# eric-downes/tianshou_marl

Measured on AMD Instinct MI355X. Metric: env-steps/sec (n_env x n_agent) incl. PPO update, simple_spread N=3, higher is better.
Workload: dtype f32; 1 GPU; simple_spread_v3 N=3 shared PPO, num_envs=1024 per GPU, obs 18, A=5, T=25, MLP 64-64; minibatch=4096, repeat=1, dispatch=per_agent, parallelism=env-shard x1

## Files before the change

tianshou_marl_amd/csrc/mlp_fused.hip:

```cpp
#include "common.h"
#include "mlp_tile.h"
#include "philox.h"

extern long long *g_tsm_stamps;

namespace {

template <int H, int DS = 0>
__global__ __launch_bounds__(NT) void policy_forward_kernel(
    const float *__restrict__ P, const float *__restrict__ img, Dims d_arg, const float *__restrict__ obs, int64_t B,
    uint64_t seed,
    uint64_t offset, const uint64_t *__restrict__ offset_dev, int mode ,
    float *__restrict__ logits_out,
    float *__restrict__ value_out, int32_t *__restrict__ act_io, float *__restrict__ logp_out) {
    extern __shared__ float lds[];
    const Dims d = DS ? dims_const(DS, 5) : d_arg;
    const Lay<H> ly(d, false);
    if (img) stage_image<H>(lds, ly, img);
    else stage_weights<H>(lds, ly, d, P);
    if (offset_dev) offset += *offset_dev;
    const int64_t n_tiles = (B + R - 1) / R;
    float xr[kXRegs];
    if ((int64_t)blockIdx.x < n_tiles) prefetch_tile_x(xr, d, obs, nullptr, 0, (int64_t)blockIdx.x * R, B);
    for (int64_t t = blockIdx.x; t < n_tiles; t += gridDim.x) {
        const int64_t row0 = t * R;
        __syncthreads();
        commit_tile_x(lds, ly.X, d, xr);
        if (t + gridDim.x < n_tiles) prefetch_tile_x(xr, d, obs, nullptr, 0, (t + gridDim.x) * R, B);
        __syncthreads();
        tile_forward<H>(lds, ly, d);
        if (logits_out) {
            for (int e = threadIdx.x; e < R * d.A; e += NT) {
                const int r = e / d.A, c = e - r * d.A;
                if (row0 + r < B) logits_out[(row0 + r) * d.A + c] = lds[ly.OUT + r * ly.ldo + c];
            }
        }
        if (threadIdx.x < R && row0 + threadIdx.x < B) {
            const int r = threadIdx.x;
            const int64_t i = row0 + r;
            const float *lg = lds + ly.OUT + r * ly.ldo;
            if (value_out) value_out[i] = lg[16];
            if (mode != 0) {
                float m = -INFINITY;
                int arg = 0;
                for (int j = 0; j < d.A; ++j) if (lg[j] > m) { m = lg[j]; arg = j; }
                float s = 0.f;
                for (int j = 0; j < d.A; ++j) s += expf(lg[j] - m);
                int a = arg;
                if (mode == 1) {
                    const float u = tsm_philox_uniform(seed, offset + (uint64_t)i) * s;
                    float c = 0.f;
                    a = d.A - 1;
                    for (int j = 0; j < d.A; ++j) { c += expf(lg[j] - m); if (u < c) { a = j; break; } }
                } else if (mode == 3) {
                    a = act_io[i];
                }
                if (mode != 3) act_io[i] = a;
                if (logp_out) logp_out[i] = lg[a] - (m + logf(s));
            }
        }
    }
}

struct LossCfg {
    float eps_clip, dual_clip, vf_coef, ent_coef;
    int value_clip, adv_norm, kind;
};

template <int H>
__global__ __launch_bounds__(NT) void ppo_update_kernel(
    const float *__restrict__ P, const float *__restrict__ img, Dims d, const float *__restrict__ obs,
    const int32_t *__restrict__ act,
    const float *__restrict__ logp_old, const float *__restrict__ adv, const float *__restrict__ returns,
    const float *__restrict__ v_s_old, const int64_t *__restrict__ perm, int64_t first, int64_t M,
    const float *__restrict__ adv_stats, LossCfg cfg, float *__restrict__ slabs,
    double *__restrict__ loss_partial, int64_t *__restrict__ opt_step_dev, long long *stamps) {
#define USTAMP(k) do { if (stamps && blockIdx.x == 0 && threadIdx.x == 0) stamps[k] = (long long)wall_clock64(); } while (0)
    extern __shared__ float lds[];
    USTAMP(0);
    if (stamps && threadIdx.x == 0 && blockIdx.x < 256) stamps[64 + 2 * blockIdx.x] = (long long)wall_clock64();
    if (opt_step_dev && blockIdx.x == 0 && threadIdx.x == 0) *opt_step_dev += 1;
    const Lay<H> ly(d, true);
    const POff<H> po(d.D, d.A);
    const int64_t n_tiles = (M + R - 1) / R;
    float xr[kXRegs];
    struct RowIn { int a_idx; float adv, logp_old, ret, v_old; } rin;
    auto row_id = [&](int64_t row0) -> int64_t {
        const int64_t i = row0 + (threadIdx.x >> 4);
        return i < M ? (perm ? perm[i] : first + i) : -1;
    };
    auto prefetch_row = [&](int64_t src) {
        rin.a_idx = 0; rin.adv = 0.f; rin.logp_old = 0.f; rin.ret = 0.f; rin.v_old = 0.f;
        if (src >= 0) {
            rin.a_idx = act[src]; rin.adv = adv[src]; rin.logp_old = logp_old[src]; rin.ret = returns[src];
            if (cfg.value_clip) rin.v_old = v_s_old[src];
        }
    };
    int64_t xs[kXRegs];
    int64_t rsrc = -1;
    const bool have_tile = (int64_t)blockIdx.x < n_tiles;
    if (have_tile) {
        prefetch_tile_ids(xs, d, perm, first, (int64_t)blockIdx.x * R, M);
        rsrc = row_id((int64_t)blockIdx.x * R);
        prefetch_tile_vals(xr, xs, obs);
        prefetch_row(rsrc);
    }
    if (img) stage_image<H>(lds, ly, img);
    else stage_weights<H>(lds, ly, d, P);
    const int lane = threadIdx.x & 63, w = threadIdx.x >> 6;
    const int r16 = lane & 15, kq = lane >> 4;
    const float invM = 1.0f / (float)M;
    float a_mean = 0.f, a_std = 1.f;
    if (cfg.adv_norm) { a_mean = adv_stats[0]; a_std = adv_stats[1]; }

    f4 g_W3a = {0.f, 0.f, 0.f, 0.f};
    f4 g_W2a[4], g_W2c[4];
    f4 g_W1a[kMaxJ], g_W1c[kMaxJ];
#pragma unroll
    for (int j = 0; j < 4; ++j) { g_W2a[j] = g_W3a; g_W2c[j] = g_W3a; }
#pragma unroll
    for (int j = 0; j < kMaxJ; ++j) { g_W1a[j] = g_W3a; g_W1c[j] = g_W3a; }
    float g_b1 = 0.f, g_b2 = 0.f;
    float g_W3c = 0.f;
    float g_b3 = 0.f;
    double s_clip = 0.0, s_vf = 0.0, s_ent = 0.0;

    for (int64_t t = blockIdx.x; t < n_tiles; t += gridDim.x) {
        const int64_t row0 = t * R;
        __syncthreads();
        USTAMP(1);
        commit_tile_x(lds, ly.X, d, xr);
        const RowIn cur = rin;
        __syncthreads();
        USTAMP(2);
        tile_forward<H>(lds, ly, d);
        USTAMP(3);

        {
            const int r = threadIdx.x >> 4, j = threadIdx.x & 15;
            const int64_t i = row0 + r;
            float *d3 = lds + ly.D3 + r * ly.ldo;
            float dl = 0.f, dv = 0.f;
            if (i < M) {
                const float *lg = lds + ly.OUT + r * ly.ldo;
                const bool on = j < d.A;
                const float x = on ? lg[j] : -INFINITY;
                const float m = row16_max(x);
                const float ex = on ? expf(x - m) : 0.f;
                const float s = row16_sum(ex);
                const float l = on ? x - (m + logf(s)) : 0.f;
                const float p = ex / s;
                const float h = row16_sum(on ? -p * l : 0.f);
                const int a_idx = cur.a_idx;
                const float logp = __shfl(l, (threadIdx.x & 48) + a_idx, 64);
                float a = cur.adv;
                if (cfg.adv_norm) a = (a - a_mean) / (a_std + 1e-8f);
                float ratio, obj, g_ratio;
                if (cfg.kind == 1) {
                    ratio = 1.f; obj = logp * a; g_ratio = a;
                } else {
                    ratio = expf(logp - cur.logp_old);
                    const float lo = 1.0f - cfg.eps_clip, hi = 1.0f + cfg.eps_clip;
                    const float rc = fminf(fmaxf(ratio, lo), hi);
                    const float s1 = ratio * a, s2 = rc * a;
                    const bool in_range = ratio >= lo && ratio <= hi;
                    if (s1 < s2) { obj = s1; g_ratio = a; }
                    else if (s1 > s2) { obj = s2; g_ratio = in_range ? a : 0.f; }
                    else { obj = s1; g_ratio = 0.5f * a + (in_range ? 0.5f * a : 0.f); }
                    if (cfg.dual_clip > 0.f && a < 0.f) {
                        const float c = cfg.dual_clip * a;
                        if (c > obj) { obj = c; g_ratio = 0.f; }
                        else if (c == obj) g_ratio *= 0.5f;
                    }
                }
                const float v = lg[16], ret = cur.ret;
                float vf, g_v;
                if (cfg.value_clip) {
                    const float vs = cur.v_old;
                    const float dd = v - vs;
                    const float dc = fminf(fmaxf(dd, -cfg.eps_clip), cfg.eps_clip);
                    const bool v_in = dd >= -cfg.eps_clip && dd <= cfg.eps_clip;
                    const float vclip = vs + dc;
                    const float vf1 = (ret - v) * (ret - v), vf2 = (ret - vclip) * (ret - vclip);
                    const float g1 = 2.f * (v - ret), g2 = v_in ? 2.f * (vclip - ret) : 0.f;
                    if (vf1 > vf2) { vf = vf1; g_v = g1; }
                    else if (vf1 < vf2) { vf = vf2; g_v = g2; }
                    else { vf = vf1; g_v = 0.5f * g1 + 0.5f * g2; }
                } else {
                    vf = (ret - v) * (ret - v);
                    g_v = 2.f * (v - ret);
                }
                dv = cfg.vf_coef * g_v * invM;
                const float g_logp = -g_ratio * ratio * invM, ec = cfg.ent_coef * invM;
                if (on) dl = g_logp * ((j == a_idx ? 1.f : 0.f) - p) + ec * p * (l + h);
                if (j == 0) { s_clip += (double)obj; s_vf += (double)vf; s_ent += (double)h; }
            }
            d3[j] = dl;
            if (j == 0) d3[16] = dv;
        }
        __syncthreads();

        if (t + gridDim.x < n_tiles) {
            prefetch_tile_x(xr, d, obs, perm, first, (t + gridDim.x) * R, M);
            prefetch_row(row_id((t + gridDim.x) * R));
        }
        USTAMP(4);
        {
            const float *dA = lds + ly.D3 + kq * ly.ldo + r16;
            const float *hB = lds + ly.H2 + kq * ly.ld2 + 16 * w + r16;
#pragma unroll
            for (int k0 = 0; k0 < R; k0 += 4) g_W3a = mfma(dA[k0 * ly.ldo], hB[k0 * ly.ld2], g_W3a);
            f4 acc = {0.f, 0.f, 0.f, 0.f};
            const float *dR = lds + ly.D3 + r16 * ly.ldo + kq;
            const float *wB = lds + ly.W3a + kq * ly.ldh + 16 * w + r16;
#pragma unroll
            for (int k0 = 0; k0 < 16; k0 += 4) acc = mfma(dR[k0], wB[k0 * ly.ldh], acc);
            const int col = 16 * w + r16;
#pragma unroll
            for (int r = 0; r < 4; ++r) {
                const int row = kq * 4 + r;
                lds[ly.D2 + row * ly.ld2 + col] = lds[ly.H2 + row * ly.ld2 + col] > 0.f ? acc[r] : 0.f;
            }
            for (int e = threadIdx.x; e < R * H; e += NT) {
                const int r = e / H, j = e - r * H;
                const float hv = lds[ly.H2 + r * ly.ld2 + H + j];
                lds[ly.D2 + r * ly.ld2 + H + j] = hv > 0.f ? lds[ly.D3 + r * ly.ldo + 16] * lds[ly.W3c + j] : 0.f;
            }
            if (threadIdx.x < H) {
                float s = 0.f;
                for (int r = 0; r < R; ++r) s = fmaf(lds[ly.D3 + r * ly.ldo + 16], lds[ly.H2 + r * ly.ld2 + H + threadIdx.x], s);
                g_W3c += s;
            }
            if (threadIdx.x < 17) {
                float s = 0.f;
                for (int r = 0; r < R; ++r) s += lds[ly.D3 + r * ly.ldo + threadIdx.x];
                g_b3 += s;
            }
        }
        __syncthreads();

        {
            const float *dAa = lds + ly.D2 + kq * ly.ld2 + 16 * w + r16;
            const float *dAc = dAa + H;
#pragma unroll
            for (int jb = 0; jb < 4; ++jb) {
                const float *hBa = lds + ly.H1 + kq * ly.ld2 + 16 * jb + r16;
                const float *hBc = hBa + H;
#pragma unroll
                for (int k0 = 0; k0 < R; k0 += 4) {
                    g_W2a[jb] = mfma(dAa[k0 * ly.ld2], hBa[k0 * ly.ld2], g_W2a[jb]);
                    g_W2c[jb] = mfma(dAc[k0 * ly.ld2], hBc[k0 * ly.ld2], g_W2c[jb]);
                }
            }
            if (threadIdx.x < 2 * H) {
                float s = 0.f;
                for (int r = 0; r < R; ++r) s += lds[ly.D2 + r * ly.ld2 + threadIdx.x];
                g_b2 += s;
            }
            f4 acc_a = {0.f, 0.f, 0.f, 0.f}, acc_c = {0.f, 0.f, 0.f, 0.f};
            const float *dRa = lds + ly.D2 + r16 * ly.ld2 + kq;
            const float *dRc = dRa + H;
            const float *wBa = lds + ly.W2a + kq * ly.ldh + 16 * w + r16;
            const float *wBc = lds + ly.W2c + kq * ly.ldh + 16 * w + r16;
#pragma unroll
            for (int k0 = 0; k0 < H; k0 += 4) {
                acc_a = mfma(dRa[k0], wBa[k0 * ly.ldh], acc_a);
                acc_c = mfma(dRc[k0], wBc[k0 * ly.ldh], acc_c);
            }
            const int col = 16 * w + r16;
#pragma unroll
            for (int r = 0; r < 4; ++r) {
                const int row = kq * 4 + r;
                lds[ly.D1 + row * ly.ld2 + col] = lds[ly.H1 + row * ly.ld2 + col] > 0.f ? acc_a[r] : 0.f;
                lds[ly.D1 + row * ly.ld2 + H + col] = lds[ly.H1 + row * ly.ld2 + H + col] > 0.f ? acc_c[r] : 0.f;
            }
        }
        __syncthreads();

        {
            const float *dAa = lds + ly.D1 + kq * ly.ld2 + 16 * w + r16;
            const float *dAc = dAa + H;
#pragma unroll
            for (int jb = 0; jb < kMaxJ; ++jb) {
                if (jb < d.nJ) {
                    const float *xB = lds + ly.X + kq * d.ld1 + 16 * jb + r16;
#pragma unroll
                    for (int k0 = 0; k0 < R; k0 += 4) {
                        const float b = xB[k0 * d.ld1];
                        g_W1a[jb] = mfma(dAa[k0 * ly.ld2], b, g_W1a[jb]);
                        g_W1c[jb] = mfma(dAc[k0 * ly.ld2], b, g_W1c[jb]);
                    }
                }
            }
            if (threadIdx.x < 2 * H) {
                float s = 0.f;
                for (int r = 0; r < R; ++r) s += lds[ly.D1 + r * ly.ld2 + threadIdx.x];
                g_b1 += s;
            }
        }
    }

    USTAMP(5);
    float *S = slabs + (int64_t)blockIdx.x * po.total;
    const int colq = r16;
#pragma unroll
    for (int r = 0; r < 4; ++r) {
        const int row = kq * 4 + r;
        if (row < d.A) __builtin_nontemporal_store(g_W3a[r], &S[po.aW3 + row * H + 16 * w + colq]);
#pragma unroll
        for (int jb = 0; jb < 4; ++jb) {
            __builtin_nontemporal_store(g_W2a[jb][r], &S[po.aW2 + (16 * w + row) * H + 16 * jb + colq]);
            __builtin_nontemporal_store(g_W2c[jb][r], &S[po.cW2 + (16 * w + row) * H + 16 * jb + colq]);
        }
#pragma unroll
        for (int jb = 0; jb < kMaxJ; ++jb) {
            const int c = 16 * jb + colq;
            if (jb < d.nJ && c < d.D) {
                __builtin_nontemporal_store(g_W1a[jb][r], &S[po.aW1 + (16 * w + row) * d.D + c]);
                __builtin_nontemporal_store(g_W1c[jb][r], &S[po.cW1 + (16 * w + row) * d.D + c]);
            }
        }
    }
    if (threadIdx.x < 2 * H) {
        const int c = threadIdx.x;
        if (c < H) { __builtin_nontemporal_store(g_b1, &S[po.ab1 + c]); __builtin_nontemporal_store(g_b2, &S[po.ab2 + c]); __builtin_nontemporal_store(g_W3c, &S[po.cW3 + c]); }
        else { __builtin_nontemporal_store(g_b1, &S[po.cb1 + c - H]); __builtin_nontemporal_store(g_b2, &S[po.cb2 + c - H]); }
    }
    if (threadIdx.x < d.A) __builtin_nontemporal_store(g_b3, &S[po.ab3 + threadIdx.x]);
    if (threadIdx.x == 16) __builtin_nontemporal_store(g_b3, &S[po.cb3]);
    {
        __shared__ double s_red[3][NT / 64];
        double c = wave_sum(s_clip), v = wave_sum(s_vf), e = wave_sum(s_ent);
        if (lane == 0) { s_red[0][w] = c; s_red[1][w] = v; s_red[2][w] = e; }
        __syncthreads();
        if (threadIdx.x == 0) {
            loss_partial[4 * blockIdx.x + 0] = s_red[0][0] + s_red[0][1] + s_red[0][2] + s_red[0][3];
            loss_partial[4 * blockIdx.x + 1] = s_red[1][0] + s_red[1][1] + s_red[1][2] + s_red[1][3];
            loss_partial[4 * blockIdx.x + 2] = s_red[2][0] + s_red[2][1] + s_red[2][2] + s_red[2][3];
            loss_partial[4 * blockIdx.x + 3] = 0.0;
        }
    }
    USTAMP(6);
    if (stamps && threadIdx.x == 0 && blockIdx.x < 256) stamps[65 + 2 * blockIdx.x] = (long long)wall_clock64();
#undef USTAMP
}

template <int H>
struct LayN {
    static constexpr int ldh = H + 2;
    static constexpr int ldo = 18;
    int W1, W2, W3, B1, B2, B3, X, H1, H2, OUT, D3, D2, D1, total;
    __host__ __device__ explicit LayN(const Dims &d) {
        int o = 0;
        W1 = o; o += H * d.ld1;
        W2 = o; o += H * ldh;
        W3 = o; o += 16 * ldh;
        B1 = o; o += H;
        B2 = o; o += H;
        B3 = o; o += 16;
        o = (o + 3) & ~3;
        X = o; o += R * d.ld1;
        H1 = o; o += R * ldh;
        H2 = o; o += R * ldh;
        OUT = o; o += R * ldo;
        D3 = o; o += R * ldo;
        D2 = o; o += R * ldh;
        D1 = o; o += R * ldh;
        total = o;
    }
};

template <int H>
struct NetImageRegs {
    static constexpr int kIt1 = (H * (16 * kMaxJ + 2) / 4 + NT - 1) / NT, kIt2 = (H * LayN<H>::ldh / 4 + NT - 1) / NT;
    static constexpr int kIt3 = (16 * LayN<H>::ldh / 4 + NT - 1) / NT;
    f4 r1[kIt1], r2[kIt2], r3[kIt3];
    float b1, b2, b3;
};

template <int H, int NET>
__device__ __forceinline__ void stage_net_image_load(NetImageRegs<H> &q, const Lay<H> &ly, const Dims &d, const float *__restrict__ img) {
    constexpr int kIt1 = NetImageRegs<H>::kIt1, kIt2 = NetImageRegs<H>::kIt2, kIt3 = NetImageRegs<H>::kIt3;
    const f4 *s1 = reinterpret_cast<const f4 *>(img + ly.W1 + NET * H * d.ld1);
    const f4 *s2 = reinterpret_cast<const f4 *>(img + (NET ? ly.W2c : ly.W2a));
    const f4 *s3 = reinterpret_cast<const f4 *>(img + (NET ? ly.W3c : ly.W3a));
    const int n1 = H * d.ld1 / 4, n2 = H * LayN<H>::ldh / 4, n3 = NET ? H / 4 : 16 * LayN<H>::ldh / 4;
#pragma unroll
    for (int it = 0; it < kIt1; ++it) { const int i = threadIdx.x + it * NT; q.r1[it] = s1[i < n1 ? i : 0]; }
#pragma unroll
    for (int it = 0; it < kIt2; ++it) { const int i = threadIdx.x + it * NT; q.r2[it] = s2[i < n2 ? i : 0]; }
#pragma unroll
    for (int it = 0; it < kIt3; ++it) { const int i = threadIdx.x + it * NT; q.r3[it] = s3[i < n3 ? i : 0]; }
    const int tb = threadIdx.x < H ? (int)threadIdx.x : 0, t3 = threadIdx.x < 16 ? (int)threadIdx.x : 0;
    q.b1 = img[ly.B1 + NET * H + tb];
    q.b2 = img[ly.B2 + NET * H + tb];
    const float b3v = img[NET ? ly.B3c : ly.B3a + t3];
    q.b3 = NET ? (threadIdx.x == 0 ? b3v : 0.f) : b3v;
}

template <int H, int NET>
__device__ __forceinline__ void stage_net_image_store(float *lds, const NetImageRegs<H> &q, const LayN<H> &ln, const Dims &d) {
    constexpr int kIt1 = NetImageRegs<H>::kIt1, kIt2 = NetImageRegs<H>::kIt2, kIt3 = NetImageRegs<H>::kIt3;
    const int n1 = H * d.ld1 / 4, n2 = H * LayN<H>::ldh / 4, n3 = NET ? H / 4 : 16 * LayN<H>::ldh / 4;
    f4 *d1 = reinterpret_cast<f4 *>(lds + ln.W1), *d2 = reinterpret_cast<f4 *>(lds + ln.W2);
    f4 *d3 = reinterpret_cast<f4 *>(lds + ln.W3);
#pragma unroll
    for (int it = 0; it < kIt1; ++it) { const int i = threadIdx.x + it * NT; if (i < n1) d1[i] = q.r1[it]; }
#pragma unroll
    for (int it = 0; it < kIt2; ++it) { const int i = threadIdx.x + it * NT; if (i < n2) d2[i] = q.r2[it]; }
#pragma unroll
    for (int it = 0; it < kIt3; ++it) { const int i = threadIdx.x + it * NT; if (i < n3) d3[i] = q.r3[it]; }
    if (threadIdx.x < H) { lds[ln.B1 + threadIdx.x] = q.b1; lds[ln.B2 + threadIdx.x] = q.b2; }
    if (threadIdx.x < 16) lds[ln.B3 + threadIdx.x] = q.b3;
}

template <int H, int NET>
__device__ __forceinline__ void stage_net_image(float *lds, const LayN<H> &ln, const Lay<H> &ly, const Dims &d,
                                                const float *__restrict__ img) {
    constexpr int kIt1 = (H * (16 * kMaxJ + 2) / 4 + NT - 1) / NT, kIt2 = (H * LayN<H>::ldh / 4 + NT - 1) / NT;
    constexpr int kIt3 = (16 * LayN<H>::ldh / 4 + NT - 1) / NT;
    const f4 *s1 = reinterpret_cast<const f4 *>(img + ly.W1 + NET * H * d.ld1);
    const f4 *s2 = reinterpret_cast<const f4 *>(img + (NET ? ly.W2c : ly.W2a));
    const f4 *s3 = reinterpret_cast<const f4 *>(img + (NET ? ly.W3c : ly.W3a));
    const int n1 = H * d.ld1 / 4, n2 = H * LayN<H>::ldh / 4, n3 = NET ? H / 4 : 16 * LayN<H>::ldh / 4;
    const f4 zero = {0.f, 0.f, 0.f, 0.f};
    f4 r1[kIt1], r2[kIt2], r3[kIt3];
#pragma unroll
    for (int it = 0; it < kIt1; ++it) { const int i = threadIdx.x + it * NT; r1[it] = i < n1 ? s1[i] : zero; }
#pragma unroll
    for (int it = 0; it < kIt2; ++it) { const int i = threadIdx.x + it * NT; r2[it] = i < n2 ? s2[i] : zero; }
#pragma unroll
    for (int it = 0; it < kIt3; ++it) { const int i = threadIdx.x + it * NT; r3[it] = i < n3 ? s3[i] : zero; }
    float b1 = 0.f, b2 = 0.f, b3 = 0.f;
    if (threadIdx.x < H) { b1 = img[ly.B1 + NET * H + threadIdx.x]; b2 = img[ly.B2 + NET * H + threadIdx.x]; }
    if (threadIdx.x < 16) b3 = NET ? (threadIdx.x == 0 ? img[ly.B3c] : 0.f) : img[ly.B3a + threadIdx.x];
    f4 *d1 = reinterpret_cast<f4 *>(lds + ln.W1), *d2 = reinterpret_cast<f4 *>(lds + ln.W2);
    f4 *d3 = reinterpret_cast<f4 *>(lds + ln.W3);
#pragma unroll
    for (int it = 0; it < kIt1; ++it) { const int i = threadIdx.x + it * NT; if (i < n1) d1[i] = r1[it]; }
#pragma unroll
    for (int it = 0; it < kIt2; ++it) { const int i = threadIdx.x + it * NT; if (i < n2) d2[i] = r2[it]; }
#pragma unroll
    for (int it = 0; it < kIt3; ++it) { const int i = threadIdx.x + it * NT; if (i < n3) d3[i] = r3[it]; }
    if (threadIdx.x < H) { lds[ln.B1 + threadIdx.x] = b1; lds[ln.B2 + threadIdx.x] = b2; }
    if (threadIdx.x < 16) lds[ln.B3 + threadIdx.x] = b3;
}

template <int H, int NET>
__device__ void stage_net_flat(float *lds, const LayN<H> &ln, const Dims &d, const float *__restrict__ P) {
    const POff<H> po(d.D, d.A);
    const int oW1 = NET ? po.cW1 : po.aW1, oW2 = NET ? po.cW2 : po.aW2, oW3 = NET ? po.cW3 : po.aW3;
    const int ob1 = NET ? po.cb1 : po.ab1, ob2 = NET ? po.cb2 : po.ab2, ob3 = NET ? po.cb3 : po.ab3;
    constexpr int U = 4;
    for (int e0 = threadIdx.x; e0 < H * d.ld1; e0 += U * NT) {
        float v[U];
#pragma unroll
        for (int u = 0; u < U; ++u) {
            const int e = e0 + u * NT, row = e / d.ld1, c = e - row * d.ld1;
            v[u] = (e < H * d.ld1 && c < d.D) ? P[oW1 + row * d.D + c] : 0.f;
        }
#pragma unroll
        for (int u = 0; u < U; ++u) if (e0 + u * NT < H * d.ld1) lds[ln.W1 + e0 + u * NT] = v[u];
    }
    for (int e0 = threadIdx.x; e0 < H * ln.ldh; e0 += U * NT) {
        float v[U];
#pragma unroll
        for (int u = 0; u < U; ++u) {
            const int e = e0 + u * NT, row = e / ln.ldh, c = e - row * ln.ldh;
            v[u] = (e < H * ln.ldh && c < H) ? P[oW2 + row * H + c] : 0.f;
        }
#pragma unroll
        for (int u = 0; u < U; ++u) if (e0 + u * NT < H * ln.ldh) lds[ln.W2 + e0 + u * NT] = v[u];
    }
    for (int e = threadIdx.x; e < 16 * ln.ldh; e += NT) {
        const int row = e / ln.ldh, c = e - row * ln.ldh;
        float v = 0.f;
        if (NET) { if (e < H) v = P[oW3 + e]; }
        else if (row < d.A && c < H) v = P[oW3 + row * H + c];
        lds[ln.W3 + e] = v;
    }
    if (threadIdx.x < H) { lds[ln.B1 + threadIdx.x] = P[ob1 + threadIdx.x]; lds[ln.B2 + threadIdx.x] = P[ob2 + threadIdx.x]; }
    if (threadIdx.x < 16) lds[ln.B3 + threadIdx.x] = threadIdx.x < (NET ? 1 : d.A) ? P[ob3 + threadIdx.x] : 0.f;
}

template <int ST>
__device__ __forceinline__ void slab_store(float v, float *p) {
    if (ST == 0) __builtin_nontemporal_store(v, p);
    else if (ST == 1) *p = v;
    else __hip_atomic_store(p, v, __ATOMIC_RELAXED, __HIP_MEMORY_SCOPE_AGENT);
}
template <int H>
constexpr int pub_floats(int ld1) { return 4 * R * H + R * ld1 + R * LayN<H>::ldo; }

__device__ __forceinline__ float column_sum(const float *col, int ld) {
    float v[R];
#pragma unroll
    for (int r = 0; r < R; ++r) v[r] = col[r * ld];
    __builtin_amdgcn_sched_barrier(0);
    float s = 0.f;
#pragma unroll
    for (int r = 0; r < R; ++r) s += v[r];
    return s;
}

template <int H, int NET, int ST, bool PUB = false, bool PK = false>
__device__ __forceinline__ void ppo_update_net(
    float *lds, const float *__restrict__ P, const float *__restrict__ img, const Dims &d, const float *__restrict__ obs,
    const int32_t *__restrict__ act, const float *__restrict__ logp_old, const float *__restrict__ adv,
    const float *__restrict__ returns, const float *__restrict__ v_s_old, const int64_t *__restrict__ perm, int64_t first,
    int64_t M, const float *__restrict__ adv_stats, const LossCfg &cfg, float *__restrict__ slabs,
    double *__restrict__ loss_partial, long long *stamps, const float *__restrict__ packed = nullptr) {
#define NSTAMP(k) do { if (stamps && blockIdx.x == 0 && threadIdx.x == 0) stamps[16 + 24 * NET + (k)] = (long long)wall_clock64(); } while (0)
    NSTAMP(0);
    if (stamps && threadIdx.x == 0 && blockIdx.x < 256) stamps[1024 + 2 * (blockIdx.x + 256 * NET)] = (long long)wall_clock64();
    const LayN<H> ln(d);
    const POff<H> po(d.D, d.A);
    const int64_t n_tiles = (M + R - 1) / R;
    float xr[kXRegs];
    struct RowIn { int a_idx; float adv, logp_old, ret, v_old; } rin;
    auto row_id = [&](int64_t row0) -> int64_t {
        const int64_t i = row0 + (threadIdx.x >> 4);
        const int64_t v = perm ? perm[i < M ? i : row0] : first + i;
        return i < M ? v : -1;
    };
    auto prefetch_row = [&](int64_t src) {
        const int64_t s0 = src >= 0 ? src : 0;
        const bool on = src >= 0;
        rin.a_idx = 0; rin.adv = 0.f; rin.logp_old = 0.f; rin.ret = 0.f; rin.v_old = 0.f;
        if (NET == 0) {
            const int a_ = act[s0]; const float ad_ = adv[s0], lp_ = logp_old[s0];
            rin.a_idx = on ? a_ : 0; rin.adv = on ? ad_ : 0.f; rin.logp_old = on ? lp_ : 0.f;
        } else {
            const float r_ = returns[s0];
            rin.ret = on ? r_ : 0.f;
            const float vo_ = (cfg.value_clip ? v_s_old : returns)[s0];
            rin.v_old = on && cfg.value_clip ? vo_ : 0.f;
        }
    };
    auto prefetch_packed = [&](int64_t t) {
        const float *rec = packed + t * pack_rec_words(d.D);
#pragma unroll
        for (int it = 0; it < kXRegs; ++it) {
            const int e = threadIdx.x + it * NT, r = e / d.ld1, c = e - r * d.ld1;
            const bool ok = e < R * d.ld1 && c < d.D;
            const float v = rec[ok ? r * d.D + c : 0];
            xr[it] = ok ? v : 0.f;
        }
        const float *row = rec + R * d.D + (threadIdx.x >> 4);
        rin.a_idx = 0; rin.adv = 0.f; rin.logp_old = 0.f; rin.ret = 0.f; rin.v_old = 0.f;
        if (NET == 0) {
            rin.a_idx = __float_as_int(row[0]); rin.logp_old = row[R]; rin.adv = row[2 * R];
        } else {
            rin.ret = row[3 * R];
            const float vo_ = row[4 * R];
            rin.v_old = cfg.value_clip ? vo_ : 0.f;
        }
    };
    if constexpr (PK) {
        static_assert(R == kPackRows, "a record is one tile");
        prefetch_packed(blockIdx.x);
        NetImageRegs<H> wq;
        const Lay<H> ly_img(d, true);
        stage_net_image_load<H, NET>(wq, ly_img, d, img);
        __builtin_amdgcn_sched_barrier(0);
        stage_net_image_store<H, NET>(lds, wq, ln, d);
    } else if (perm && img && (int64_t)blockIdx.x < n_tiles) {
        int64_t xs[kXRegs], id0[kXRegs + 1];
        prefetch_tile_ids_load<1>(id0, d, perm, first, (int64_t)blockIdx.x * R, M);
        NetImageRegs<H> wq;
        const Lay<H> ly_img(d, true);
        stage_net_image_load<H, NET>(wq, ly_img, d, img);
        __builtin_amdgcn_sched_barrier(0);
        unsigned ok;
        const int64_t rsrc = prefetch_tile_ids_done_nb(xs, ok, id0, d, (int64_t)blockIdx.x * R, M);
        prefetch_tile_vals_nb(xr, xs, ok, obs);
        prefetch_row(rsrc);
        __builtin_amdgcn_sched_barrier(0);
        stage_net_image_store<H, NET>(lds, wq, ln, d);
    } else {
        int64_t xs[kXRegs];
        if ((int64_t)blockIdx.x < n_tiles) {
            prefetch_tile_ids(xs, d, perm, first, (int64_t)blockIdx.x * R, M);
            const int64_t rsrc = row_id((int64_t)blockIdx.x * R);
            prefetch_tile_vals(xr, xs, obs);
            prefetch_row(rsrc);
        }
        if (img) { const Lay<H> ly(d, true); stage_net_image<H, NET>(lds, ln, ly, d, img); }
        else stage_net_flat<H, NET>(lds, ln, d, P);
    }
    const int lane = threadIdx.x & 63, w = threadIdx.x >> 6;
    const int r16 = lane & 15, kq = lane >> 4;
    const float invM = 1.0f / (float)M;
    float a_mean = 0.f, a_std = 1.f;
    if (NET == 0 && cfg.adv_norm) { a_mean = adv_stats[0]; a_std = adv_stats[1]; }

    const f4 zero = {0.f, 0.f, 0.f, 0.f};
    f4 g_W3 = zero;
    f4 g_W2[4], g_W1[kMaxJ];
#pragma unroll
    for (int j = 0; j < 4; ++j) g_W2[j] = zero;
#pragma unroll
    for (int j = 0; j < kMaxJ; ++j) g_W1[j] = zero;
    float g_b1 = 0.f, g_b2 = 0.f;
    float g_W3c = 0.f;
    float g_b3 = 0.f;
    double s_a = 0.0, s_b = 0.0;

    float *const S = slabs + (int64_t)blockIdx.x * po.total;
    auto store_out_layer = [&]() {
        if constexpr (!PUB) {
            if (NET == 0) {
#pragma unroll
                for (int r = 0; r < 4; ++r) {
                    const int row = kq * 4 + r;
                    if (row < d.A) slab_store<ST>(g_W3[r], &S[po.aW3 + row * H + 16 * w + r16]);
                }
                if (threadIdx.x < d.A) slab_store<ST>(g_b3, &S[po.ab3 + threadIdx.x]);
            } else {
                if (threadIdx.x < H) slab_store<ST>(g_W3c, &S[po.cW3 + threadIdx.x]);
                if (threadIdx.x == 0) slab_store<ST>(g_b3, &S[po.cb3]);
            }
        }
    };
    auto store_layer2 = [&]() {
        if constexpr (!PUB) {
            const int oW2 = NET ? po.cW2 : po.aW2;
#pragma unroll
            for (int r = 0; r < 4; ++r)
#pragma unroll
                for (int jb = 0; jb < 4; ++jb) slab_store<ST>(g_W2[jb][r], &S[oW2 + (16 * w + kq * 4 + r) * H + 16 * jb + r16]);
            if (threadIdx.x < H) slab_store<ST>(g_b2, &S[(NET ? po.cb2 : po.ab2) + threadIdx.x]);
        }
    };
    auto store_layer1 = [&]() {
        if constexpr (!PUB) {
            const int oW1 = NET ? po.cW1 : po.aW1;
#pragma unroll
            for (int r = 0; r < 4; ++r)
#pragma unroll
                for (int jb = 0; jb < kMaxJ; ++jb) {
                    const int c = 16 * jb + r16;
                    if (jb < d.nJ && c < d.D) slab_store<ST>(g_W1[jb][r], &S[oW1 + (16 * w + kq * 4 + r) * d.D + c]);
                }
            if (threadIdx.x < H) slab_store<ST>(g_b1, &S[(NET ? po.cb1 : po.ab1) + threadIdx.x]);
        }
    };
    bool stored = false;
    NSTAMP(1);
    for (int64_t t = blockIdx.x; t < n_tiles; t += gridDim.x) {
        const int64_t row0 = t * R;
        const bool last_tile = t + gridDim.x >= n_tiles;
        __syncthreads();
        commit_tile_x(lds, ln.X, d, xr);
        const RowIn cur = rin;
        __syncthreads();
        NSTAMP(2);
        {
            f4 acc = zero;
            const float *xa = lds + ln.X + r16 * d.ld1 + kq;
            const float *wa = lds + ln.W1 + (16 * w + r16) * d.ld1 + kq;
            for (int k0 = 0; k0 < d.Kp1; k0 += 4) acc = mfma(xa[k0], wa[k0], acc);
            const int col = 16 * w + r16;
            const float b = lds[ln.B1 + col];
#pragma unroll
            for (int r = 0; r < 4; ++r) lds[ln.H1 + (kq * 4 + r) * ln.ldh + col] = fmaxf(acc[r] + b, 0.f);
        }
        __syncthreads();
        NSTAMP(3);
        {
            f4 acc = zero;
            const float *ha = lds + ln.H1 + r16 * ln.ldh + kq;
            const float *wa = lds + ln.W2 + (16 * w + r16) * ln.ldh + kq;
#pragma unroll
            for (int k0 = 0; k0 < H; k0 += 4) acc = mfma(ha[k0], wa[k0], acc);
            const int col = 16 * w + r16;
            const float b = lds[ln.B2 + col];
#pragma unroll
            for (int r = 0; r < 4; ++r) lds[ln.H2 + (kq * 4 + r) * ln.ldh + col] = fmaxf(acc[r] + b, 0.f);
        }
        __syncthreads();
        NSTAMP(4);
        if (NET == 0) {
            if (w == 0) {
                f4 acc = zero;
                const float *ha = lds + ln.H2 + r16 * ln.ldh + kq;
                const float *wa = lds + ln.W3 + r16 * ln.ldh + kq;
#pragma unroll
                for (int k0 = 0; k0 < H; k0 += 4) acc = mfma(ha[k0], wa[k0], acc);
                const float b = lds[ln.B3 + r16];
#pragma unroll
                for (int r = 0; r < 4; ++r) lds[ln.OUT + (kq * 4 + r) * ln.ldo + r16] = acc[r] + b;
            }
        } else if (threadIdx.x < R) {
            const float sv = fmaf_chain_ahead<H>(lds + ln.H2 + threadIdx.x * ln.ldh, lds + ln.W3);
            lds[ln.OUT + threadIdx.x * ln.ldo + 16] = sv + lds[ln.B3];
        }
        __syncthreads();
        NSTAMP(5);

        {
            const int r = threadIdx.x >> 4, j = threadIdx.x & 15;
            const int64_t i = row0 + r;
            float *d3 = lds + ln.D3 + r * ln.ldo;
            float dl = 0.f, dv = 0.f;
            if (i < M) {
                const float *lg = lds + ln.OUT + r * ln.ldo;
                if (NET == 0) {
                    const bool on = j < d.A;
                    const float x = on ? lg[j] : -INFINITY;
                    const float m = row16_max(x);
                    const float ex = on ? expf(x - m) : 0.f;
                    const float s = row16_sum(ex);
                    const float l = on ? x - (m + logf(s)) : 0.f;
                    const float p = ex / s;
                    const float h = row16_sum(on ? -p * l : 0.f);
                    const int a_idx = cur.a_idx;
                    const float logp = __shfl(l, (threadIdx.x & 48) + a_idx, 64);
                    float a = cur.adv;
                    if (cfg.adv_norm) a = (a - a_mean) / (a_std + 1e-8f);
                    float ratio, obj, g_ratio;
                    if (cfg.kind == 1) {
                        ratio = 1.f; obj = logp * a; g_ratio = a;
                    } else {
                        ratio = expf(logp - cur.logp_old);
                        const float lo = 1.0f - cfg.eps_clip, hi = 1.0f + cfg.eps_clip;
                        const float rc = fminf(fmaxf(ratio, lo), hi);
                        const float s1 = ratio * a, s2 = rc * a;
                        const bool in_range = ratio >= lo && ratio <= hi;
                        if (s1 < s2) { obj = s1; g_ratio = a; }
                        else if (s1 > s2) { obj = s2; g_ratio = in_range ? a : 0.f; }
                        else { obj = s1; g_ratio = 0.5f * a + (in_range ? 0.5f * a : 0.f); }
                        if (cfg.dual_clip > 0.f && a < 0.f) {
                            const float c = cfg.dual_clip * a;
                            if (c > obj) { obj = c; g_ratio = 0.f; }
                            else if (c == obj) g_ratio *= 0.5f;
                        }
                    }
                    const float g_logp = -g_ratio * ratio * invM, ec = cfg.ent_coef * invM;
                    if (on) dl = g_logp * ((j == a_idx ? 1.f : 0.f) - p) + ec * p * (l + h);
                    if (j == 0) { s_a += (double)obj; s_b += (double)h; }
                } else if (j == 0) {
                    const float v = lg[16], ret = cur.ret;
                    float vf, g_v;
                    if (cfg.value_clip) {
                        const float vs = cur.v_old;
                        const float dd = v - vs;
                        const float dc = fminf(fmaxf(dd, -cfg.eps_clip), cfg.eps_clip);
                        const bool v_in = dd >= -cfg.eps_clip && dd <= cfg.eps_clip;
                        const float vclip = vs + dc;
                        const float vf1 = (ret - v) * (ret - v), vf2 = (ret - vclip) * (ret - vclip);
                        const float g1 = 2.f * (v - ret), g2 = v_in ? 2.f * (vclip - ret) : 0.f;
                        if (vf1 > vf2) { vf = vf1; g_v = g1; }
                        else if (vf1 < vf2) { vf = vf2; g_v = g2; }
                        else { vf = vf1; g_v = 0.5f * g1 + 0.5f * g2; }
                    } else {
                        vf = (ret - v) * (ret - v);
                        g_v = 2.f * (v - ret);
                    }
                    dv = cfg.vf_coef * g_v * invM;
                    s_a += (double)vf;
                }
            }
            if (NET == 0) d3[j] = dl;
            else if (j == 0) d3[16] = dv;
        }
        __syncthreads();
        NSTAMP(6);

        if (t + gridDim.x < n_tiles) {
            if constexpr (PK) prefetch_packed(t + gridDim.x);
            else {
                prefetch_tile_x(xr, d, obs, perm, first, (t + gridDim.x) * R, M);
                prefetch_row(row_id((t + gridDim.x) * R));
            }
        }
        if (NET == 0) {
            const float *dA = lds + ln.D3 + kq * ln.ldo + r16;
            const float *hB = lds + ln.H2 + kq * ln.ldh + 16 * w + r16;
            if constexpr (!PUB) {
#pragma unroll
                for (int k0 = 0; k0 < R; k0 += 4) g_W3 = mfma(dA[k0 * ln.ldo], hB[k0 * ln.ldh], g_W3);
            }
            f4 acc = zero;
            const float *dR = lds + ln.D3 + r16 * ln.ldo + kq;
            const float *wB = lds + ln.W3 + kq * ln.ldh + 16 * w + r16;
#pragma unroll
            for (int k0 = 0; k0 < 16; k0 += 4) acc = mfma(dR[k0], wB[k0 * ln.ldh], acc);
            const int col = 16 * w + r16;
#pragma unroll
            for (int r = 0; r < 4; ++r) {
                const int row = kq * 4 + r;
                lds[ln.D2 + row * ln.ldh + col] = lds[ln.H2 + row * ln.ldh + col] > 0.f ? acc[r] : 0.f;
            }
            if (!PUB && threadIdx.x < 16) g_b3 += column_sum(lds + ln.D3 + threadIdx.x, ln.ldo);
        } else {
            static_assert(NT == 4 * H && R == 16, "one column per lane, four rows per wave");
            const int j = threadIdx.x & (H - 1);
            float d4[4], h4[4], dv[R], hcol[R];
#pragma unroll
            for (int k = 0; k < 4; ++k) { d4[k] = lds[ln.D3 + (4 * k + w) * ln.ldo + 16]; h4[k] = lds[ln.H2 + (4 * k + w) * ln.ldh + j]; }
            const float w3j = lds[ln.W3 + j];
            if (!PUB && w == 0) {
#pragma unroll
                for (int r = 0; r < R; ++r) { dv[r] = lds[ln.D3 + r * ln.ldo + 16]; hcol[r] = lds[ln.H2 + r * ln.ldh + j]; }
            }
            __builtin_amdgcn_sched_barrier(0);
#pragma unroll
            for (int k = 0; k < 4; ++k) lds[ln.D2 + (4 * k + w) * ln.ldh + j] = h4[k] > 0.f ? d4[k] * w3j : 0.f;
            if (!PUB && w == 0) {
                float s = 0.f;
#pragma unroll
                for (int r = 0; r < R; ++r) s = fmaf(dv[r], hcol[r], s);
                g_W3c += s;
                if (threadIdx.x == 0) {
                    float sb = 0.f;
#pragma unroll
                    for (int r = 0; r < R; ++r) sb += dv[r];
                    g_b3 += sb;
                }
            }
        }
        if (last_tile) { store_out_layer(); stored = true; }
        __syncthreads();
        NSTAMP(7);
        {
            const float *dA = lds + ln.D2 + kq * ln.ldh + 16 * w + r16;
            if constexpr (!PUB) {
#pragma unroll
                for (int jb = 0; jb < 4; ++jb) {
                    const float *hB = lds + ln.H1 + kq * ln.ldh + 16 * jb + r16;
#pragma unroll
                    for (int k0 = 0; k0 < R; k0 += 4) g_W2[jb] = mfma(dA[k0 * ln.ldh], hB[k0 * ln.ldh], g_W2[jb]);
                }
                if (threadIdx.x < H) g_b2 += column_sum(lds + ln.D2 + threadIdx.x, ln.ldh);
                if (last_tile) store_layer2();
            }
            f4 acc = zero;
            const float *dR = lds + ln.D2 + r16 * ln.ldh + kq;
            const float *wB = lds + ln.W2 + kq * ln.ldh + 16 * w + r16;
#pragma unroll
            for (int k0 = 0; k0 < H; k0 += 4) acc = mfma(dR[k0], wB[k0 * ln.ldh], acc);
            const int col = 16 * w + r16;
#pragma unroll
            for (int r = 0; r < 4; ++r) {
                const int row = kq * 4 + r;
                lds[ln.D1 + row * ln.ldh + col] = lds[ln.H1 + row * ln.ldh + col] > 0.f ? acc[r] : 0.f;
            }
        }
        __syncthreads();
        NSTAMP(8);
        if constexpr (PUB) {
            float *pub = slabs + ((int64_t)t * 2 + NET) * pub_floats<H>(d.ld1);
            const int pr = threadIdx.x >> 4, pc = (threadIdx.x & 15) * 4;
            const int src[4] = {ln.H1, ln.H2, ln.D2, ln.D1};
#pragma unroll
            for (int m = 0; m < 4; ++m) {
                const float2 a0 = *reinterpret_cast<const float2 *>(lds + src[m] + pr * ln.ldh + pc);
                const float2 a1 = *reinterpret_cast<const float2 *>(lds + src[m] + pr * ln.ldh + pc + 2);
                __builtin_nontemporal_store(f4{a0.x, a0.y, a1.x, a1.y}, reinterpret_cast<f4 *>(pub + m * R * H + pr * H + pc));
            }
            for (int e = threadIdx.x; e < R * d.ld1; e += NT) __builtin_nontemporal_store(lds[ln.X + e], pub + 4 * R * H + e);
            for (int e = threadIdx.x; e < R * ln.ldo; e += NT) __builtin_nontemporal_store(lds[ln.D3 + e], pub + 4 * R * H + R * d.ld1 + e);
        } else
        {
            const float *dA = lds + ln.D1 + kq * ln.ldh + 16 * w + r16;
#pragma unroll
            for (int jb = 0; jb < kMaxJ; ++jb) {
                if (jb < d.nJ) {
                    const float *xB = lds + ln.X + kq * d.ld1 + 16 * jb + r16;
#pragma unroll
                    for (int k0 = 0; k0 < R; k0 += 4) g_W1[jb] = mfma(dA[k0 * ln.ldh], xB[k0 * d.ld1], g_W1[jb]);
                }
            }
            if (threadIdx.x < H) g_b1 += column_sum(lds + ln.D1 + threadIdx.x, ln.ldh);
        }
    }

    NSTAMP(9);
    if (!stored) { store_out_layer(); store_layer2(); }
    store_layer1();
    NSTAMP(10);
    {
        __shared__ double s_red[2][NT / 64];
        const double a = wave_sum(s_a), b = wave_sum(s_b);
        if (lane == 0) { s_red[0][w] = a; s_red[1][w] = b; }
        __syncthreads();
        if (threadIdx.x == 0) {
            const double ta = s_red[0][0] + s_red[0][1] + s_red[0][2] + s_red[0][3];
            const double tb = s_red[1][0] + s_red[1][1] + s_red[1][2] + s_red[1][3];
            if (NET == 0) {
                loss_partial[4 * blockIdx.x + 0] = ta;
                loss_partial[4 * blockIdx.x + 2] = tb;
                loss_partial[4 * blockIdx.x + 3] = 0.0;
            } else {
                loss_partial[4 * blockIdx.x + 1] = ta;
            }
            NSTAMP(11);
            if (stamps && blockIdx.x < 256) stamps[1025 + 2 * (blockIdx.x + 256 * NET)] = (long long)wall_clock64();
        }
    }
#undef NSTAMP
}

template <int H, int ST, int DS, bool PUB = false, bool PK = false>
__global__ __launch_bounds__(NT, 2) void ppo_update_split_kernel(

    const float *__restrict__ P, const float *__restrict__ img, Dims d_arg, const float *__restrict__ obs,
    const int32_t *__restrict__ act, const float *__restrict__ logp_old, const float *__restrict__ adv,
    const float *__restrict__ returns, const float *__restrict__ v_s_old, const int64_t *__restrict__ perm, int64_t first,
    int64_t M, const float *__restrict__ adv_stats, LossCfg cfg, float *__restrict__ slabs,
    double *__restrict__ loss_partial, int64_t *__restrict__ opt_step_dev, long long *stamps, const float *__restrict__ packed) {
    extern __shared__ float lds[];
    const Dims d = DS ? dims_const(DS, 5) : d_arg;
    if (opt_step_dev && blockIdx.x == 0 && blockIdx.y == 0 && threadIdx.x == 0) *opt_step_dev += 1;
    if (blockIdx.y == 0)
        ppo_update_net<H, 0, ST, PUB, PK>(lds, P, img, d, obs, act, logp_old, adv, returns, v_s_old, perm, first, M, adv_stats, cfg,
                                          slabs, loss_partial, stamps, packed);
    else
        ppo_update_net<H, 1, ST, PUB, PK>(lds, P, img, d, obs, act, logp_old, adv, returns, v_s_old, perm, first, M, adv_stats, cfg,
                                          slabs, loss_partial, stamps, packed);
}

__global__ __launch_bounds__(256) void update_finalize_kernel(const double *__restrict__ partial, int n_blocks,
                                                              int64_t M, float vf_coef, float ent_coef,
                                                              float *__restrict__ scalars) {
    __shared__ double sm[256 / 64];
    double c = 0.0, v = 0.0, e = 0.0;
    for (int b = threadIdx.x; b < n_blocks; b += 256) {
        c += partial[4 * b + 0];
        v += partial[4 * b + 1];
        e += partial[4 * b + 2];
    }
    c = block_sum<double, 256>(c, sm);
    v = block_sum<double, 256>(v, sm);
    e = block_sum<double, 256>(e, sm);
    if (threadIdx.x == 0) {
        const double clip_loss = -c / (double)M, vf_loss = v / (double)M, ent_loss = e / (double)M;
        scalars[0] = (float)(clip_loss + (double)vf_coef * vf_loss - (double)ent_coef * ent_loss);
        scalars[1] = (float)clip_loss;
        scalars[2] = (float)vf_loss;
        scalars[3] = (float)ent_loss;
    }
}

__global__ __launch_bounds__(256) void update_finalize_many_kernel(const double *__restrict__ partial,
                                                                   int64_t stride_elems,
                                                                   const int32_t *__restrict__ n_blocks,
                                                                   const int64_t *__restrict__ M, float vf_coef,
                                                                   float ent_coef, float *__restrict__ scalars) {
    __shared__ double sm[256 / 64];
    const int k = blockIdx.x;
    const double *p = partial + (int64_t)k * stride_elems;
    double c = 0.0, v = 0.0, e = 0.0;
    for (int b = threadIdx.x; b < n_blocks[k]; b += 256) {
        c += p[4 * b + 0];
        v += p[4 * b + 1];
        e += p[4 * b + 2];
    }
    c = block_sum<double, 256>(c, sm);
    v = block_sum<double, 256>(v, sm);
    e = block_sum<double, 256>(e, sm);
    if (threadIdx.x == 0) {
        const double m = (double)M[k];
        const double clip_loss = -c / m, vf_loss = v / m, ent_loss = e / m;
        scalars[4 * k + 0] = (float)(clip_loss + (double)vf_coef * vf_loss - (double)ent_coef * ent_loss);
        scalars[4 * k + 1] = (float)clip_loss;
        scalars[4 * k + 2] = (float)vf_loss;
        scalars[4 * k + 3] = (float)ent_loss;
    }
}

}

TSM_EXPORT int64_t tsm_policy_param_count(int32_t obs_dim, int32_t hidden, int32_t n_act) {
    if (hidden != 64) return -1;
    return POff<64>(obs_dim, n_act).total;
}

TSM_EXPORT int64_t tsm_policy_image_elems(int32_t obs_dim, int32_t hidden, int32_t n_act) {
    Dims d;
    if (make_dims(obs_dim, hidden, n_act, &d)) return -1;
    const Lay<64> ly(d, false);
    const int64_t padded = (int64_t)image_f4_padded(ly.X) * 4;
    return padded <= ly.total ? padded : -1;
}

TSM_EXPORT int tsm_policy_image_map(int32_t obs_dim, int32_t hidden, int32_t n_act, int32_t *map_out_host) {
    Dims d;
    if (int rc = make_dims(obs_dim, hidden, n_act, &d)) return rc;
    TSM_REQUIRE(map_out_host, "tsm_policy_image_map: null pointer");
    constexpr int H = 64;
    const Lay<H> ly(d, false);
    const POff<H> po(d.D, d.A);
    int32_t *m = map_out_host;
    for (int r = 0; r < H; ++r)
        for (int c = 0; c < d.D; ++c) {
            m[po.aW1 + r * d.D + c] = ly.W1 + r * d.ld1 + c;
            m[po.cW1 + r * d.D + c] = ly.W1 + (H + r) * d.ld1 + c;
        }
    for (int r = 0; r < H; ++r)
        for (int c = 0; c < H; ++c) {
            m[po.aW2 + r * H + c] = ly.W2a + r * ly.ldh + c;
            m[po.cW2 + r * H + c] = ly.W2c + r * ly.ldh + c;
        }
    for (int r = 0; r < d.A; ++r)
        for (int c = 0; c < H; ++c) m[po.aW3 + r * H + c] = ly.W3a + r * ly.ldh + c;
    for (int c = 0; c < H; ++c) {
        m[po.cW3 + c] = ly.W3c + c;
        m[po.ab1 + c] = ly.B1 + c;
        m[po.cb1 + c] = ly.B1 + H + c;
        m[po.ab2 + c] = ly.B2 + c;
        m[po.cb2 + c] = ly.B2 + H + c;
    }
    for (int c = 0; c < d.A; ++c) m[po.ab3 + c] = ly.B3a + c;
    m[po.cb3] = ly.B3c;
    return TSM_OK;
}

TSM_EXPORT int tsm_policy_forward(const float *params, const float *param_image, int32_t obs_dim, int32_t hidden,
                                  int32_t n_act,
                                  const float *obs, int64_t B, int mode, uint64_t seed, uint64_t offset,
                                  const uint64_t *offset_dev, float *logits_out, float *value_out, int32_t *act_io, float *logp_out,
                                  void *stream) {
    Dims d;
    if (int rc = make_dims(obs_dim, hidden, n_act, &d)) return rc;
    TSM_REQUIRE(B >= 0 && mode >= 0 && mode <= 3, "tsm_policy_forward: bad B / mode");
    if (B == 0) return TSM_OK;
    TSM_REQUIRE(params && obs, "tsm_policy_forward: null pointer");
    TSM_REQUIRE(mode == 0 || act_io, "tsm_policy_forward: mode %d needs act_io", mode);
    const Lay<64> ly(d, false);
    const size_t shmem = (size_t)ly.total * sizeof(float);
    const int64_t n_tiles = ceil_div(B, R);
    unsigned grid = (unsigned)(n_tiles < 512 ? n_tiles : 512);
    static bool attr_set = false;
    if (!attr_set) {
        TSM_HIP(tsm_allow_max_lds(reinterpret_cast<const void *>(policy_forward_kernel<64>)));
        TSM_HIP(tsm_allow_max_lds(reinterpret_cast<const void *>(policy_forward_kernel<64, 18>)));
        TSM_HIP(tsm_allow_max_lds(reinterpret_cast<const void *>(policy_forward_kernel<64, 16>)));
        attr_set = true;
    }
    const bool spec = d.A == 5 && !tsm_opt(TSM_OPT_GENERIC);
    auto kern = (spec && d.D == 18) ? policy_forward_kernel<64, 18> : (spec && d.D == 16) ? policy_forward_kernel<64, 16> : policy_forward_kernel<64>;
    hipLaunchKernelGGL(kern, dim3(grid), dim3(NT), shmem, tsm_stream(stream), params,
                       param_image, d, obs,
                       B, seed, offset, offset_dev, mode, logits_out, value_out, act_io, logp_out);
    TSM_LAUNCH_CHECK();
    return TSM_OK;
}

static int g_update_variant = 0;
static int g_slab_store = 0;
extern "C" __attribute__((visibility("default"))) void tsm_debug_set_slab_store(int v) { g_slab_store = v; }
extern "C" __attribute__((visibility("default"))) void tsm_debug_set_update_variant(int v) { g_update_variant = v; }
extern "C" int tsm_debug_update_variant_get(void) { return g_update_variant; }
extern "C" int tsm_debug_slab_store_get(void) { return g_slab_store; }

TSM_EXPORT int tsm_ppo_update_grid(int64_t M, int32_t max_blocks) {
    const int64_t n_tiles = ceil_div(M > 0 ? M : 1, R);
    int64_t g;
    if (n_tiles <= 256) g = n_tiles;
    else if (n_tiles < 1024) g = (n_tiles + 1) / 2 < 256 ? (n_tiles + 1) / 2 : 256;
    else g = 384;
    if (max_blocks > 0 && g > max_blocks) g = max_blocks;
    return (int)g;
}

TSM_EXPORT int tsm_ppo_update_fused_packed(const float *params, const float *param_image, int32_t obs_dim, int32_t hidden,
                                           int32_t n_act,
                                           const float *obs, const int32_t *act, const float *logp_old, const float *adv,
                                           const float *returns, const float *v_s_old, const int64_t *perm,
                                           int64_t first_row, int64_t M, const float *adv_stats,
                                           const tsm_ppo_cfg *cfg_host, int32_t n_blocks, float *grad_slabs_out,
                                           double *loss_partial_out, float *scalars_out, int64_t *opt_step_dev,
                                           const float *packed, void *stream) {
    Dims d;
    if (int rc = make_dims(obs_dim, hidden, n_act, &d)) return rc;
    TSM_REQUIRE(M >= 1, "tsm_ppo_update_fused: M must be >= 1");
    TSM_REQUIRE(cfg_host && params && obs && act && logp_old && adv && returns && grad_slabs_out && loss_partial_out,
                "tsm_ppo_update_fused: null pointer");
    TSM_REQUIRE(!cfg_host->value_clip || v_s_old, "tsm_ppo_update_fused: value_clip needs v_s_old");
    TSM_REQUIRE(!cfg_host->adv_norm || adv_stats, "tsm_ppo_update_fused: adv_norm needs adv_stats");
    TSM_REQUIRE(cfg_host->loss_kind == 0 || cfg_host->loss_kind == 1, "tsm_ppo_update_fused: loss_kind must be 0 or 1");
    TSM_REQUIRE(cfg_host->dual_clip <= 0.0 || cfg_host->dual_clip > 1.0,
                "Dual-clip PPO parameter should greater than 1.0 but got %g", cfg_host->dual_clip);
    TSM_REQUIRE(n_blocks >= 1 && n_blocks <= ceil_div(M, R), "tsm_ppo_update_fused: n_blocks=%d out of range",
                n_blocks);
    LossCfg cfg;
    cfg.eps_clip = (float)cfg_host->eps_clip;
    cfg.dual_clip = (float)cfg_host->dual_clip;
    cfg.vf_coef = (float)cfg_host->vf_coef;
    cfg.ent_coef = (float)cfg_host->ent_coef;
    cfg.value_clip = cfg_host->value_clip;
    cfg.adv_norm = cfg_host->adv_norm;
    cfg.kind = cfg_host->loss_kind;
    const Lay<64> ly(d, true);
    const size_t shmem = (size_t)ly.total * sizeof(float);
    static bool attr_set = false;
    if (!attr_set) {
        TSM_HIP(tsm_allow_max_lds(reinterpret_cast<const void *>(ppo_update_kernel<64>)));
        attr_set = true;
    }
    hipStream_t st = tsm_stream(stream);
    if (g_update_variant == 2) {
        TSM_REQUIRE(d.D == 18 && d.A == 5 && (int64_t)n_blocks == ceil_div(M, R) && param_image,
                    "update variant 2 (kernel A timing) serves the headline shape only: obs 18, 5 actions, one tile per workgroup, image");
        const LayN<64> ln(d);
        hipLaunchKernelGGL((ppo_update_split_kernel<64, 0, 18, true>), dim3((unsigned)n_blocks, 2), dim3(NT),
                           (size_t)ln.total * sizeof(float), st, params, param_image, d, obs, act, logp_old, adv, returns,
                           v_s_old, perm, first_row, M, adv_stats, cfg, grad_slabs_out, loss_partial_out, opt_step_dev, g_tsm_stamps,
                           (const float *)nullptr);
    } else if (g_update_variant == 0) {
        const LayN<64> ln(d);
        const bool spec = d.A == 5 && !tsm_opt(TSM_OPT_GENERIC);
        const bool pk = packed && param_image && g_slab_store == 0;
        auto kern = g_slab_store == 1 ? ppo_update_split_kernel<64, 1, 0>
                    : g_slab_store == 2 ? ppo_update_split_kernel<64, 2, 0>
                    : (spec && d.D == 18) ? (pk ? ppo_update_split_kernel<64, 0, 18, false, true>
                                                : ppo_update_split_kernel<64, 0, 18>)
                    : (spec && d.D == 16) ? (pk ? ppo_update_split_kernel<64, 0, 16, false, true>
                                                : ppo_update_split_kernel<64, 0, 16>)
                    : pk ? ppo_update_split_kernel<64, 0, 0, false, true> : ppo_update_split_kernel<64, 0, 0>;
        hipLaunchKernelGGL(kern, dim3((unsigned)n_blocks, 2), dim3(NT),
                           (size_t)ln.total * sizeof(float), st, params, param_image, d, obs, act, logp_old, adv, returns,
                           v_s_old, perm, first_row, M, adv_stats, cfg, grad_slabs_out, loss_partial_out, opt_step_dev, g_tsm_stamps,
                           pk ? packed : nullptr);
    } else {
        hipLaunchKernelGGL((ppo_update_kernel<64>), dim3((unsigned)n_blocks), dim3(NT), shmem, st, params, param_image, d,
                           obs, act,
                           logp_old, adv, returns, v_s_old, perm, first_row, M, adv_stats, cfg, grad_slabs_out,
                           loss_partial_out, opt_step_dev, g_tsm_stamps);
    }
    TSM_LAUNCH_CHECK();
    if (scalars_out) {
        hipLaunchKernelGGL(update_finalize_kernel, dim3(1), dim3(256), 0, st, loss_partial_out, n_blocks, M,
                           cfg.vf_coef, cfg.ent_coef, scalars_out);
        TSM_LAUNCH_CHECK();
    }
    return TSM_OK;
}

TSM_EXPORT int tsm_ppo_update_fused(const float *params, const float *param_image, int32_t obs_dim, int32_t hidden,
                                    int32_t n_act,
                                    const float *obs, const int32_t *act, const float *logp_old, const float *adv,
                                    const float *returns, const float *v_s_old, const int64_t *perm,
                                    int64_t first_row, int64_t M, const float *adv_stats,
                                    const tsm_ppo_cfg *cfg_host, int32_t n_blocks, float *grad_slabs_out,
                                    double *loss_partial_out, float *scalars_out, int64_t *opt_step_dev,
                                    void *stream) {
    return tsm_ppo_update_fused_packed(params, param_image, obs_dim, hidden, n_act, obs, act, logp_old, adv, returns, v_s_old, perm,
                                       first_row, M, adv_stats, cfg_host, n_blocks, grad_slabs_out, loss_partial_out, scalars_out,
                                       opt_step_dev, nullptr, stream);
}

TSM_EXPORT int tsm_ppo_finalize_many(const double *partial, int64_t stride_elems, const int32_t *n_blocks_dev,
                                     const int64_t *M_dev, int32_t n_steps, const tsm_ppo_cfg *cfg_host,
                                     float *scalars_out, void *stream) {
    TSM_REQUIRE(n_steps >= 0, "tsm_ppo_finalize_many: negative n_steps");
    if (n_steps == 0) return TSM_OK;
    TSM_REQUIRE(partial && n_blocks_dev && M_dev && cfg_host && scalars_out && stride_elems >= 4,
                "tsm_ppo_finalize_many: bad args");
    hipLaunchKernelGGL(update_finalize_many_kernel, dim3((unsigned)n_steps), dim3(256), 0, tsm_stream(stream), partial,
                       stride_elems, n_blocks_dev, M_dev, (float)cfg_host->vf_coef, (float)cfg_host->ent_coef,
                       scalars_out);
    TSM_LAUNCH_CHECK();
    return TSM_OK;
}
```

tianshou_marl_amd/csrc/mlp_tile.h:

```cpp
#pragma once
#include "common.h"

namespace {

typedef float f4 __attribute__((ext_vector_type(4)));

constexpr int R = 16;
constexpr int NT = 256;
constexpr int kMaxJ = 4;

struct Dims {
    int D, A;
    int Kp1;
    int nJ;
    int ld1;
};

__host__ __device__ constexpr Dims dims_const(int D, int A) {
    Dims d{};
    d.D = D; d.A = A; d.Kp1 = (D + 3) / 4 * 4; d.nJ = (D + 15) / 16; d.ld1 = 16 * ((D + 15) / 16) + 2;
    return d;
}

template <int H>
struct Lay {
    static constexpr int ldh = H + 2;
    static constexpr int ld2 = 2 * H + 2;
    static constexpr int ldo = 18;
    int W1, W2a, W2c, W3a, W3c, B1, B2, B3a, B3c, X, H1, H2, OUT, D3, D2, D1, total;
    __host__ __device__ Lay(const Dims &d, bool bwd) {
        int o = 0;
        W1 = o; o += 2 * H * d.ld1;
        W2a = o; o += H * ldh;
        W2c = o; o += H * ldh;
        W3a = o; o += 16 * ldh;
        W3c = o; o += H;
        B1 = o; o += 2 * H;
        B2 = o; o += 2 * H;
        B3a = o; o += 16;
        B3c = o; o += 2;
        o = (o + 3) & ~3;
        X = o; o += R * d.ld1;
        H1 = o; o += R * ld2;
        H2 = o; o += R * ld2;
        OUT = o; o += R * ldo;
        D3 = o; o += bwd ? R * ldo : 0;
        D2 = o; o += bwd ? R * ld2 : 0;
        D1 = o; o += bwd ? R * ld2 : 0;
        total = o;
    }
};

__device__ __forceinline__ f4 mfma(float a, float b, f4 c) {
    return __builtin_amdgcn_mfma_f32_16x16x4f32(a, b, c, 0, 0, 0);
}

template <int N>
__device__ __forceinline__ float fmaf_chain_ahead(const float *h, const float *w) {
    constexpr int Q = 8;
    static_assert(N % (2 * Q) == 0, "pairs of whole groups");
    float h0[Q], w0[Q], h1[Q], w1[Q], s = 0.f;
    int off = 0;
    auto pin = [&]() { asm volatile("" : "+v"(s), "+v"(off)); };
#pragma unroll
    for (int p = 0; p < Q; ++p) { h0[p] = h[p]; w0[p] = w[p]; }
#pragma unroll
    for (int j0 = 0; j0 < N; j0 += 2 * Q) {
        pin();
#pragma unroll
        for (int p = 0; p < Q; ++p) { h1[p] = h[off + j0 + Q + p]; w1[p] = w[off + j0 + Q + p]; }
#pragma unroll
        for (int p = 0; p < Q; ++p) s = fmaf(h0[p], w0[p], s);
        pin();
        if (j0 + 2 * Q < N) {
#pragma unroll
            for (int p = 0; p < Q; ++p) { h0[p] = h[off + j0 + 2 * Q + p]; w0[p] = w[off + j0 + 2 * Q + p]; }
        }
#pragma unroll
        for (int p = 0; p < Q; ++p) s = fmaf(h1[p], w1[p], s);
    }
    return s;
}

template <int H>
struct POff {
    int aW1, ab1, aW2, ab2, aW3, ab3, cW1, cb1, cW2, cb2, cW3, cb3, total;
    __host__ __device__ POff(int D, int A) {
        int o = 0;
        aW1 = o; o += H * D; ab1 = o; o += H; aW2 = o; o += H * H; ab2 = o; o += H; aW3 = o; o += A * H; ab3 = o; o += A;
        cW1 = o; o += H * D; cb1 = o; o += H; cW2 = o; o += H * H; cb2 = o; o += H; cW3 = o; o += H; cb3 = o; o += 1;
        total = o;
    }
};

template <int H>
__device__ void stage_weights(float *lds, const Lay<H> &ly, const Dims &d, const float *__restrict__ P, int tid_in = -1) {
    const POff<H> po(d.D, d.A);
    const int tid = tid_in < 0 ? (int)threadIdx.x : tid_in;
    constexpr int U = 12;
    for (int e0 = tid; e0 < 2 * H * d.ld1; e0 += U * NT) {
        float v[U];
#pragma unroll
        for (int u = 0; u < U; ++u) {
            const int e = e0 + u * NT;
            const int row = e / d.ld1, c = e - row * d.ld1;
            v[u] = 0.f;
            if (e < 2 * H * d.ld1 && c < d.D) v[u] = row < H ? P[po.aW1 + row * d.D + c] : P[po.cW1 + (row - H) * d.D + c];
        }
#pragma unroll
        for (int u = 0; u < U; ++u)
            if (e0 + u * NT < 2 * H * d.ld1) lds[ly.W1 + e0 + u * NT] = v[u];
    }
    for (int e0 = tid; e0 < H * ly.ldh; e0 += U * NT) {
        float va[U], vc[U];
#pragma unroll
        for (int u = 0; u < U; ++u) {
            const int e = e0 + u * NT;
            const int row = e / ly.ldh, c = e - row * ly.ldh;
            const bool on = e < H * ly.ldh && c < H;
            va[u] = on ? P[po.aW2 + row * H + c] : 0.f;
            vc[u] = on ? P[po.cW2 + row * H + c] : 0.f;
        }
#pragma unroll
        for (int u = 0; u < U; ++u) {
            const int e = e0 + u * NT;
            if (e < H * ly.ldh) { lds[ly.W2a + e] = va[u]; lds[ly.W2c + e] = vc[u]; }
        }
    }
    {
        constexpr int N3 = (16 * Lay<H>::ldh + NT - 1) / NT;
        float v3[N3], vv[5];
#pragma unroll
        for (int u = 0; u < N3; ++u) {
            const int e = tid + u * NT, row = e / ly.ldh, c = e - row * ly.ldh;
            v3[u] = (e < 16 * ly.ldh && row < d.A && c < H) ? P[po.aW3 + row * H + c] : 0.f;
        }
        const int e5 = tid < H ? tid : 0;
        vv[0] = P[po.cW3 + e5]; vv[1] = P[po.ab1 + e5]; vv[2] = P[po.cb1 + e5]; vv[3] = P[po.ab2 + e5]; vv[4] = P[po.cb2 + e5];
#pragma unroll
        for (int u = 0; u < N3; ++u) {
            const int e = tid + u * NT;
            if (e < 16 * ly.ldh) lds[ly.W3a + e] = v3[u];
        }
        if (tid < H) {
            lds[ly.W3c + tid] = vv[0]; lds[ly.B1 + tid] = vv[1]; lds[ly.B1 + H + tid] = vv[2]; lds[ly.B2 + tid] = vv[3];
            lds[ly.B2 + H + tid] = vv[4];
        }
    }
    if (tid < 16) lds[ly.B3a + tid] = tid < d.A ? P[po.ab3 + tid] : 0.f;
    if (tid == 0) lds[ly.B3c] = P[po.cb3];
}

constexpr int kStageChunk = 4 * 256;
__host__ __device__ inline int image_f4_padded(int x_floats) {
    return ((x_floats / 4) + kStageChunk - 1) / kStageChunk * kStageChunk;
}

template <int H>
__device__ __forceinline__ void stage_image(float *lds, const Lay<H> &ly, const float *__restrict__ img) {
    const int n4p = image_f4_padded(ly.X);
    const int wave_base = (threadIdx.x >> 6) * 64;
    for (int e = 0; e < n4p; e += NT) {
        __builtin_amdgcn_global_load_lds(
            (const __attribute__((address_space(1))) void *)(img + (size_t)(e + threadIdx.x) * 4),
            (__attribute__((address_space(3))) void *)(lds + (size_t)(e + wave_base) * 4), 16, 0, 0);
    }
}

template <int H>
__device__ __forceinline__ void tile_forward(float *lds, const Lay<H> &ly, const Dims &d) {
    const int lane = threadIdx.x & 63, w = threadIdx.x >> 6;
    const int r16 = lane & 15, kq = lane >> 4;
    {
        f4 acc_a = {0.f, 0.f, 0.f, 0.f}, acc_c = {0.f, 0.f, 0.f, 0.f};
        const float *xa = lds + ly.X + r16 * d.ld1 + kq;
        const float *wa = lds + ly.W1 + (16 * w + r16) * d.ld1 + kq;
        const float *wc = lds + ly.W1 + (H + 16 * w + r16) * d.ld1 + kq;
        for (int k0 = 0; k0 < d.Kp1; k0 += 4) {
            const float a = xa[k0];
            acc_a = mfma(a, wa[k0], acc_a);
            acc_c = mfma(a, wc[k0], acc_c);
        }
        const int col = 16 * w + r16;
        const float ba = lds[ly.B1 + col], bc = lds[ly.B1 + H + col];
#pragma unroll
        for (int r = 0; r < 4; ++r) {
            const int row = kq * 4 + r;
            lds[ly.H1 + row * ly.ld2 + col] = fmaxf(acc_a[r] + ba, 0.f);
            lds[ly.H1 + row * ly.ld2 + H + col] = fmaxf(acc_c[r] + bc, 0.f);
        }
    }
    __syncthreads();
    {
        f4 acc_a = {0.f, 0.f, 0.f, 0.f}, acc_c = {0.f, 0.f, 0.f, 0.f};
        const float *ha = lds + ly.H1 + r16 * ly.ld2 + kq;
        const float *hc = ha + H;
        const float *wa = lds + ly.W2a + (16 * w + r16) * ly.ldh + kq;
        const float *wc = lds + ly.W2c + (16 * w + r16) * ly.ldh + kq;
#pragma unroll
        for (int k0 = 0; k0 < H; k0 += 4) {
            acc_a = mfma(ha[k0], wa[k0], acc_a);
            acc_c = mfma(hc[k0], wc[k0], acc_c);
        }
        const int col = 16 * w + r16;
        const float ba = lds[ly.B2 + col], bc = lds[ly.B2 + H + col];
#pragma unroll
        for (int r = 0; r < 4; ++r) {
            const int row = kq * 4 + r;
            lds[ly.H2 + row * ly.ld2 + col] = fmaxf(acc_a[r] + ba, 0.f);
            lds[ly.H2 + row * ly.ld2 + H + col] = fmaxf(acc_c[r] + bc, 0.f);
        }
    }
    __syncthreads();
    if (w == 0) {
        f4 acc = {0.f, 0.f, 0.f, 0.f};
        const float *ha = lds + ly.H2 + r16 * ly.ld2 + kq;
        const float *wa = lds + ly.W3a + r16 * ly.ldh + kq;
#pragma unroll
        for (int k0 = 0; k0 < H; k0 += 4) acc = mfma(ha[k0], wa[k0], acc);
        const float b = lds[ly.B3a + r16];
#pragma unroll
        for (int r = 0; r < 4; ++r) lds[ly.OUT + (kq * 4 + r) * ly.ldo + r16] = acc[r] + b;
    } else if (w == 1 && lane < R) {
        const float *hc = lds + ly.H2 + lane * ly.ld2 + H;
        float s = 0.f;
        for (int j = 0; j < H; ++j) s = fmaf(hc[j], lds[ly.W3c + j], s);
        lds[ly.OUT + lane * ly.ldo + 16] = s + lds[ly.B3c];
    }
    __syncthreads();
}

template <int H>
__device__ __forceinline__ void tile_forward_split(float *lds, const Lay<H> &ly, const Dims &d) {
    const int lane = threadIdx.x & 63, w8 = threadIdx.x >> 6, net = w8 >> 2, w = w8 & 3;
    const int r16 = lane & 15, kq = lane >> 4;
    const int col = 16 * w + r16;
    {
        f4 acc = {0.f, 0.f, 0.f, 0.f};
        const float *xa = lds + ly.X + r16 * d.ld1 + kq;
        const float *wp = lds + ly.W1 + (net * H + col) * d.ld1 + kq;
        for (int k0 = 0; k0 < d.Kp1; k0 += 4) acc = mfma(xa[k0], wp[k0], acc);
        const float b = lds[ly.B1 + net * H + col];
#pragma unroll
        for (int r = 0; r < 4; ++r) lds[ly.H1 + (kq * 4 + r) * ly.ld2 + net * H + col] = fmaxf(acc[r] + b, 0.f);
    }
    __syncthreads();
    {
        f4 acc = {0.f, 0.f, 0.f, 0.f};
        const float *ha = lds + ly.H1 + r16 * ly.ld2 + net * H + kq;
        const float *wp = lds + (net ? ly.W2c : ly.W2a) + col * ly.ldh + kq;
#pragma unroll
        for (int k0 = 0; k0 < H; k0 += 4) acc = mfma(ha[k0], wp[k0], acc);
        const float b = lds[ly.B2 + net * H + col];
#pragma unroll
        for (int r = 0; r < 4; ++r) lds[ly.H2 + (kq * 4 + r) * ly.ld2 + net * H + col] = fmaxf(acc[r] + b, 0.f);
    }
    __syncthreads();
    if (w8 == 0) {
        f4 acc = {0.f, 0.f, 0.f, 0.f};
        const float *ha = lds + ly.H2 + r16 * ly.ld2 + kq;
        const float *wa = lds + ly.W3a + r16 * ly.ldh + kq;
#pragma unroll
        for (int k0 = 0; k0 < H; k0 += 4) acc = mfma(ha[k0], wa[k0], acc);
        const float b = lds[ly.B3a + r16];
#pragma unroll
        for (int r = 0; r < 4; ++r) lds[ly.OUT + (kq * 4 + r) * ly.ldo + r16] = acc[r] + b;
    } else if (w8 == 5 && lane < R) {
        const float *hc = lds + ly.H2 + lane * ly.ld2 + H;
        float s = 0.f;
        for (int j = 0; j < H; ++j) s = fmaf(hc[j], lds[ly.W3c + j], s);
        lds[ly.OUT + lane * ly.ldo + 16] = s + lds[ly.B3c];
    }
    __syncthreads();
}

constexpr int kXRegs = (R * (16 * kMaxJ + 2) + NT - 1) / NT;

template <int HAS_PERM = -1>
__device__ __forceinline__ void prefetch_tile_ids_load(int64_t (&id)[kXRegs + 1], const Dims &d, const int64_t *__restrict__ perm,
                                                       int64_t first, int64_t row0, int64_t M) {
    const int64_t ir = row0 + (threadIdx.x >> 4);
    if (HAS_PERM == 1 || (HAS_PERM == -1 && perm)) {
#pragma unroll
        for (int it = 0; it < kXRegs; ++it) {
            const int e = threadIdx.x + it * NT, r = e / d.ld1;
            const int64_t i = row0 + r;
            id[it] = perm[(e < R * d.ld1 && i < M) ? i : row0];
        }
        id[kXRegs] = perm[ir < M ? ir : row0];
    } else {
#pragma unroll
        for (int it = 0; it < kXRegs; ++it) id[it] = first + row0 + (threadIdx.x + it * NT) / d.ld1;
        id[kXRegs] = first + ir;
    }
}
__device__ __forceinline__ int64_t prefetch_tile_ids_done(int64_t (&xs)[kXRegs], const int64_t (&id)[kXRegs + 1], const Dims &d,
                                                          int64_t row0, int64_t M) {
#pragma unroll
    for (int it = 0; it < kXRegs; ++it) {
        const int e = threadIdx.x + it * NT, r = e / d.ld1, c = e - r * d.ld1;
        xs[it] = (e < R * d.ld1 && c < d.D && row0 + r < M) ? id[it] * d.D + c : -1;
    }
    return row0 + (threadIdx.x >> 4) < M ? id[kXRegs] : -1;
}
__device__ __forceinline__ int64_t prefetch_tile_ids_done_nb(int64_t (&xs)[kXRegs], unsigned &ok, const int64_t (&id)[kXRegs + 1],
                                                             const Dims &d, int64_t row0, int64_t M) {
    ok = 0;
#pragma unroll
    for (int it = 0; it < kXRegs; ++it) {
        const int e = threadIdx.x + it * NT, r = e / d.ld1, c = e - r * d.ld1;
        xs[it] = id[it] * d.D + (c < d.D ? c : 0);
        ok |= (unsigned)(e < R * d.ld1 && c < d.D && row0 + r < M) << it;
    }
    return row0 + (threadIdx.x >> 4) < M ? id[kXRegs] : -1;
}
__device__ __forceinline__ void prefetch_tile_vals_nb(float (&xr)[kXRegs], const int64_t (&xs)[kXRegs], unsigned ok,
                                                      const float *__restrict__ obs) {
#pragma unroll
    for (int it = 0; it < kXRegs; ++it) {
        const float v = obs[xs[it]];
        xr[it] = (ok >> it & 1u) ? v : 0.f;
    }
}
__device__ __forceinline__ void prefetch_tile_ids(int64_t (&xs)[kXRegs], const Dims &d,
                                                  const int64_t *__restrict__ perm, int64_t first, int64_t row0,
                                                  int64_t M) {
    int64_t id[kXRegs + 1];
    prefetch_tile_ids_load(id, d, perm, first, row0, M);
    (void)prefetch_tile_ids_done(xs, id, d, row0, M);
}

__device__ __forceinline__ void prefetch_tile_vals(float (&xr)[kXRegs], const int64_t (&xs)[kXRegs],
                                                   const float *__restrict__ obs) {
#pragma unroll
    for (int it = 0; it < kXRegs; ++it) {
        const float v = obs[xs[it] >= 0 ? xs[it] : 0];
        xr[it] = xs[it] >= 0 ? v : 0.f;
    }
}

__device__ __forceinline__ void prefetch_tile_x(float (&xr)[kXRegs], const Dims &d, const float *__restrict__ obs,
                                                const int64_t *__restrict__ perm, int64_t first, int64_t row0,
                                                int64_t M) {
    int64_t xs[kXRegs];
    prefetch_tile_ids(xs, d, perm, first, row0, M);
    prefetch_tile_vals(xr, xs, obs);
}

__device__ __forceinline__ void commit_tile_x(float *lds, int X, const Dims &d, const float (&xr)[kXRegs]) {
#pragma unroll
    for (int it = 0; it < kXRegs; ++it) {
        const int e = threadIdx.x + it * NT;
        if (e < R * d.ld1) lds[X + e] = xr[it];
    }
}

__device__ __forceinline__ void load_tile_x(float *lds, int X, const Dims &d, const float *__restrict__ obs,
                                            const int64_t *__restrict__ perm, int64_t first, int64_t row0,
                                            int64_t M) {
    float xr[kXRegs];
    prefetch_tile_x(xr, d, obs, perm, first, row0, M);
    commit_tile_x(lds, X, d, xr);
}

static int make_dims(int32_t obs_dim, int32_t hidden, int32_t n_act, Dims *d) {
    TSM_REQUIRE(hidden == 64, "fused MLP supports hidden == 64 (got %d)", hidden);
    TSM_REQUIRE(obs_dim >= 1 && obs_dim <= 16 * kMaxJ, "fused MLP supports 1 <= obs_dim <= %d (got %d)", 16 * kMaxJ,
                obs_dim);
    TSM_REQUIRE(n_act >= 1 && n_act <= 16, "fused MLP supports 1 <= n_act <= 16 (got %d)", n_act);
    d->D = obs_dim;
    d->A = n_act;
    d->Kp1 = (obs_dim + 3) / 4 * 4;
    d->nJ = (obs_dim + 15) / 16;
    d->ld1 = 16 * d->nJ + 2;
    return TSM_OK;
}


}
```

Baseline: 166.5 million env-steps/s.

## Process two tiles per workgroup in PPO update with paired reduction

Adds a pair form of the PPO update. Each workgroup runs 2*NT threads, and its two halves work on interleaved tiles side by side, sharing one staged weight image in LDS while keeping separate activation and gradient regions. Gradient accumulators are folded through extra LDS scratch. For the non-split variants, a path launches two strided kernels followed by a fold kernel. The intent is to spread weight staging over more rows and raise occupancy or parallelism when there are few tiles per block, at the cost of more LDS, more registers and an extra reduction step.

```diff
diff --git a/tianshou_marl_amd/csrc/mlp_fused.hip b/tianshou_marl_amd/csrc/mlp_fused.hip
--- a/tianshou_marl_amd/csrc/mlp_fused.hip
+++ b/tianshou_marl_amd/csrc/mlp_fused.hip
@@ -74,7 +74,7 @@
     const float *__restrict__ logp_old, const float *__restrict__ adv, const float *__restrict__ returns,
     const float *__restrict__ v_s_old, const int64_t *__restrict__ perm, int64_t first, int64_t M,
     const float *__restrict__ adv_stats, LossCfg cfg, float *__restrict__ slabs,
-    double *__restrict__ loss_partial, int64_t *__restrict__ opt_step_dev, long long *stamps) {
+    double *__restrict__ loss_partial, int64_t *__restrict__ opt_step_dev, long long *stamps, int tile_mul, int tile_add) {
 #define USTAMP(k) do { if (stamps && blockIdx.x == 0 && threadIdx.x == 0) stamps[k] = (long long)wall_clock64(); } while (0)
     extern __shared__ float lds[];
     USTAMP(0);
@@ -98,10 +98,11 @@
     };
     int64_t xs[kXRegs];
     int64_t rsrc = -1;
-    const bool have_tile = (int64_t)blockIdx.x < n_tiles;
+    auto tile_of = [&](int64_t u) -> int64_t { return u * tile_mul + tile_add; };
+    const bool have_tile = tile_of(blockIdx.x) < n_tiles;
     if (have_tile) {
-        prefetch_tile_ids(xs, d, perm, first, (int64_t)blockIdx.x * R, M);
-        rsrc = row_id((int64_t)blockIdx.x * R);
+        prefetch_tile_ids(xs, d, perm, first, tile_of(blockIdx.x) * R, M);
+        rsrc = row_id(tile_of(blockIdx.x) * R);
         prefetch_tile_vals(xr, xs, obs);
         prefetch_row(rsrc);
     }
@@ -125,8 +126,8 @@
     float g_b3 = 0.f;
     double s_clip = 0.0, s_vf = 0.0, s_ent = 0.0;
 
-    for (int64_t t = blockIdx.x; t < n_tiles; t += gridDim.x) {
-        const int64_t row0 = t * R;
+    for (int64_t u = blockIdx.x; tile_of(u) < n_tiles; u += gridDim.x) {
+        const int64_t t = tile_of(u), tn = tile_of(u + gridDim.x), row0 = t * R;
         __syncthreads();
         USTAMP(1);
         commit_tile_x(lds, ly.X, d, xr);
@@ -200,9 +201,9 @@
         }
         __syncthreads();
 
-        if (t + gridDim.x < n_tiles) {
-            prefetch_tile_x(xr, d, obs, perm, first, (t + gridDim.x) * R, M);
-            prefetch_row(row_id((t + gridDim.x) * R));
+        if (tn < n_tiles) {
+            prefetch_tile_x(xr, d, obs, perm, first, tn * R, M);
+            prefetch_row(row_id(tn * R));
         }
         USTAMP(4);
         {
@@ -371,26 +372,42 @@
 };
 
 template <int H>
+struct PairEx {
+    int W3, B3, W2, B2, W1, B1, total;
+    __host__ __device__ PairEx(const LayN<H> &ln, int nJ) {
+        int o = ln.total + (ln.total - ln.X);
+        o = (o + 3) & ~3;
+        W3 = o; o += 4 * NT;
+        W2 = o; o += 4 * 4 * NT;
+        W1 = o; o += 4 * nJ * NT;
+        B3 = o; o += 16;
+        B2 = o; o += H;
+        B1 = o; o += H;
+        total = o;
+    }
+};
+
+template <int H, int NTH = NT>
 struct NetImageRegs {
-    static constexpr int kIt1 = (H * (16 * kMaxJ + 2) / 4 + NT - 1) / NT, kIt2 = (H * LayN<H>::ldh / 4 + NT - 1) / NT;
-    static constexpr int kIt3 = (16 * LayN<H>::ldh / 4 + NT - 1) / NT;
+    static constexpr int kIt1 = (H * (16 * kMaxJ + 2) / 4 + NTH - 1) / NTH, kIt2 = (H * LayN<H>::ldh / 4 + NTH - 1) / NTH;
+    static constexpr int kIt3 = (16 * LayN<H>::ldh / 4 + NTH - 1) / NTH;
     f4 r1[kIt1], r2[kIt2], r3[kIt3];
     float b1, b2, b3;
 };
 
-template <int H, int NET>
-__device__ __forceinline__ void stage_net_image_load(NetImageRegs<H> &q, const Lay<H> &ly, const Dims &d, const float *__restrict__ img) {
-    constexpr int kIt1 = NetImageRegs<H>::kIt1, kIt2 = NetImageRegs<H>::kIt2, kIt3 = NetImageRegs<H>::kIt3;
+template <int H, int NET, int NTH = NT>
+__device__ __forceinline__ void stage_net_image_load(NetImageRegs<H, NTH> &q, const Lay<H> &ly, const Dims &d, const float *__restrict__ img) {
+    constexpr int kIt1 = NetImageRegs<H, NTH>::kIt1, kIt2 = NetImageRegs<H, NTH>::kIt2, kIt3 = NetImageRegs<H, NTH>::kIt3;
     const f4 *s1 = reinterpret_cast<const f4 *>(img + ly.W1 + NET * H * d.ld1);
     const f4 *s2 = reinterpret_cast<const f4 *>(img + (NET ? ly.W2c : ly.W2a));
     const f4 *s3 = reinterpret_cast<const f4 *>(img + (NET ? ly.W3c : ly.W3a));
     const int n1 = H * d.ld1 / 4, n2 = H * LayN<H>::ldh / 4, n3 = NET ? H / 4 : 16 * LayN<H>::ldh / 4;
 #pragma unroll
-    for (int it = 0; it < kIt1; ++it) { const int i = threadIdx.x + it * NT; q.r1[it] = s1[i < n1 ? i : 0]; }
-#pragma unroll
-    for (int it = 0; it < kIt2; ++it) { const int i = threadIdx.x + it * NT; q.r2[it] = s2[i < n2 ? i : 0]; }
-#pragma unroll
-    for (int it = 0; it < kIt3; ++it) { const int i = threadIdx.x + it * NT; q.r3[it] = s3[i < n3 ? i : 0]; }
+    for (int it = 0; it < kIt1; ++it) { const int i = threadIdx.x + it * NTH; q.r1[it] = s1[i < n1 ? i : 0]; }
+#pragma unroll
+    for (int it = 0; it < kIt2; ++it) { const int i = threadIdx.x + it * NTH; q.r2[it] = s2[i < n2 ? i : 0]; }
+#pragma unroll
+    for (int it = 0; it < kIt3; ++it) { const int i = threadIdx.x + it * NTH; q.r3[it] = s3[i < n3 ? i : 0]; }
     const int tb = threadIdx.x < H ? (int)threadIdx.x : 0, t3 = threadIdx.x < 16 ? (int)threadIdx.x : 0;
     q.b1 = img[ly.B1 + NET * H + tb];
     q.b2 = img[ly.B2 + NET * H + tb];
@@ -398,27 +415,27 @@
     q.b3 = NET ? (threadIdx.x == 0 ? b3v : 0.f) : b3v;
 }
 
-template <int H, int NET>
-__device__ __forceinline__ void stage_net_image_store(float *lds, const NetImageRegs<H> &q, const LayN<H> &ln, const Dims &d) {
-    constexpr int kIt1 = NetImageRegs<H>::kIt1, kIt2 = NetImageRegs<H>::kIt2, kIt3 = NetImageRegs<H>::kIt3;
+template <int H, int NET, int NTH = NT>
+__device__ __forceinline__ void stage_net_image_store(float *lds, const NetImageRegs<H, NTH> &q, const LayN<H> &ln, const Dims &d) {
+    constexpr int kIt1 = NetImageRegs<H, NTH>::kIt1, kIt2 = NetImageRegs<H, NTH>::kIt2, kIt3 = NetImageRegs<H, NTH>::kIt3;
     const int n1 = H * d.ld1 / 4, n2 = H * LayN<H>::ldh / 4, n3 = NET ? H / 4 : 16 * LayN<H>::ldh / 4;
     f4 *d1 = reinterpret_cast<f4 *>(lds + ln.W1), *d2 = reinterpret_cast<f4 *>(lds + ln.W2);
     f4 *d3 = reinterpret_cast<f4 *>(lds + ln.W3);
 #pragma unroll
-    for (int it = 0; it < kIt1; ++it) { const int i = threadIdx.x + it * NT; if (i < n1) d1[i] = q.r1[it]; }
-#pragma unroll
-    for (int it = 0; it < kIt2; ++it) { const int i = threadIdx.x + it * NT; if (i < n2) d2[i] = q.r2[it]; }
-#pragma unroll
-    for (int it = 0; it < kIt3; ++it) { const int i = threadIdx.x + it * NT; if (i < n3) d3[i] = q.r3[it]; }
+    for (int it = 0; it < kIt1; ++it) { const int i = threadIdx.x + it * NTH; if (i < n1) d1[i] = q.r1[it]; }
+#pragma unroll
+    for (int it = 0; it < kIt2; ++it) { const int i = threadIdx.x + it * NTH; if (i < n2) d2[i] = q.r2[it]; }
+#pragma unroll
+    for (int it = 0; it < kIt3; ++it) { const int i = threadIdx.x + it * NTH; if (i < n3) d3[i] = q.r3[it]; }
     if (threadIdx.x < H) { lds[ln.B1 + threadIdx.x] = q.b1; lds[ln.B2 + threadIdx.x] = q.b2; }
     if (threadIdx.x < 16) lds[ln.B3 + threadIdx.x] = q.b3;
 }
 
-template <int H, int NET>
+template <int H, int NET, int NTH = NT>
 __device__ __forceinline__ void stage_net_image(float *lds, const LayN<H> &ln, const Lay<H> &ly, const Dims &d,
                                                 const float *__restrict__ img) {
-    constexpr int kIt1 = (H * (16 * kMaxJ + 2) / 4 + NT - 1) / NT, kIt2 = (H * LayN<H>::ldh / 4 + NT - 1) / NT;
-    constexpr int kIt3 = (16 * LayN<H>::ldh / 4 + NT - 1) / NT;
+    constexpr int kIt1 = (H * (16 * kMaxJ + 2) / 4 + NTH - 1) / NTH, kIt2 = (H * LayN<H>::ldh / 4 + NTH - 1) / NTH;
+    constexpr int kIt3 = (16 * LayN<H>::ldh / 4 + NTH - 1) / NTH;
     const f4 *s1 = reinterpret_cast<const f4 *>(img + ly.W1 + NET * H * d.ld1);
     const f4 *s2 = reinterpret_cast<const f4 *>(img + (NET ? ly.W2c : ly.W2a));
     const f4 *s3 = reinterpret_cast<const f4 *>(img + (NET ? ly.W3c : ly.W3a));
@@ -426,53 +443,53 @@
     const f4 zero = {0.f, 0.f, 0.f, 0.f};
     f4 r1[kIt1], r2[kIt2], r3[kIt3];
 #pragma unroll
-    for (int it = 0; it < kIt1; ++it) { const int i = threadIdx.x + it * NT; r1[it] = i < n1 ? s1[i] : zero; }
-#pragma unroll
-    for (int it = 0; it < kIt2; ++it) { const int i = threadIdx.x + it * NT; r2[it] = i < n2 ? s2[i] : zero; }
-#pragma unroll
-    for (int it = 0; it < kIt3; ++it) { const int i = threadIdx.x + it * NT; r3[it] = i < n3 ? s3[i] : zero; }
+    for (int it = 0; it < kIt1; ++it) { const int i = threadIdx.x + it * NTH; r1[it] = i < n1 ? s1[i] : zero; }
+#pragma unroll
+    for (int it = 0; it < kIt2; ++it) { const int i = threadIdx.x + it * NTH; r2[it] = i < n2 ? s2[i] : zero; }
+#pragma unroll
+    for (int it = 0; it < kIt3; ++it) { const int i = threadIdx.x + it * NTH; r3[it] = i < n3 ? s3[i] : zero; }
     float b1 = 0.f, b2 = 0.f, b3 = 0.f;
     if (threadIdx.x < H) { b1 = img[ly.B1 + NET * H + threadIdx.x]; b2 = img[ly.B2 + NET * H + threadIdx.x]; }
     if (threadIdx.x < 16) b3 = NET ? (threadIdx.x == 0 ? img[ly.B3c] : 0.f) : img[ly.B3a + threadIdx.x];
     f4 *d1 = reinterpret_cast<f4 *>(lds + ln.W1), *d2 = reinterpret_cast<f4 *>(lds + ln.W2);
     f4 *d3 = reinterpret_cast<f4 *>(lds + ln.W3);
 #pragma unroll
-    for (int it = 0; it < kIt1; ++it) { const int i = threadIdx.x + it * NT; if (i < n1) d1[i] = r1[it]; }
-#pragma unroll
-    for (int it = 0; it < kIt2; ++it) { const int i = threadIdx.x + it * NT; if (i < n2) d2[i] = r2[it]; }
-#pragma unroll
-    for (int it = 0; it < kIt3; ++it) { const int i = threadIdx.x + it * NT; if (i < n3) d3[i] = r3[it]; }
+    for (int it = 0; it < kIt1; ++it) { const int i = threadIdx.x + it * NTH; if (i < n1) d1[i] = r1[it]; }
+#pragma unroll
+    for (int it = 0; it < kIt2; ++it) { const int i = threadIdx.x + it * NTH; if (i < n2) d2[i] = r2[it]; }
+#pragma unroll
+    for (int it = 0; it < kIt3; ++it) { const int i = threadIdx.x + it * NTH; if (i < n3) d3[i] = r3[it]; }
     if (threadIdx.x < H) { lds[ln.B1 + threadIdx.x] = b1; lds[ln.B2 + threadIdx.x] = b2; }
     if (threadIdx.x < 16) lds[ln.B3 + threadIdx.x] = b3;
 }
 
-template <int H, int NET>
+template <int H, int NET, int NTH = NT>
 __device__ void stage_net_flat(float *lds, const LayN<H> &ln, const Dims &d, const float *__restrict__ P) {
     const POff<H> po(d.D, d.A);
     const int oW1 = NET ? po.cW1 : po.aW1, oW2 = NET ? po.cW2 : po.aW2, oW3 = NET ? po.cW3 : po.aW3;
     const int ob1 = NET ? po.cb1 : po.ab1, ob2 = NET ? po.cb2 : po.ab2, ob3 = NET ? po.cb3 : po.ab3;
     constexpr int U = 4;
-    for (int e0 = threadIdx.x; e0 < H * d.ld1; e0 += U * NT) {
+    for (int e0 = threadIdx.x; e0 < H * d.ld1; e0 += U * NTH) {
         float v[U];
 #pragma unroll
         for (int u = 0; u < U; ++u) {
-            const int e = e0 + u * NT, row = e / d.ld1, c = e - row * d.ld1;
+            const int e = e0 + u * NTH, row = e / d.ld1, c = e - row * d.ld1;
             v[u] = (e < H * d.ld1 && c < d.D) ? P[oW1 + row * d.D + c] : 0.f;
         }
 #pragma unroll
-        for (int u = 0; u < U; ++u) if (e0 + u * NT < H * d.ld1) lds[ln.W1 + e0 + u * NT] = v[u];
-    }
-    for (int e0 = threadIdx.x; e0 < H * ln.ldh; e0 += U * NT) {
+        for (int u = 0; u < U; ++u) if (e0 + u * NTH < H * d.ld1) lds[ln.W1 + e0 + u * NTH] = v[u];
+    }
+    for (int e0 = threadIdx.x; e0 < H * ln.ldh; e0 += U * NTH) {
         float v[U];
 #pragma unroll
         for (int u = 0; u < U; ++u) {
-            const int e = e0 + u * NT, row = e / ln.ldh, c = e - row * ln.ldh;
+            const int e = e0 + u * NTH, row = e / ln.ldh, c = e - row * ln.ldh;
             v[u] = (e < H * ln.ldh && c < H) ? P[oW2 + row * H + c] : 0.f;
         }
 #pragma unroll
-        for (int u = 0; u < U; ++u) if (e0 + u * NT < H * ln.ldh) lds[ln.W2 + e0 + u * NT] = v[u];
-    }
-    for (int e = threadIdx.x; e < 16 * ln.ldh; e += NT) {
+        for (int u = 0; u < U; ++u) if (e0 + u * NTH < H * ln.ldh) lds[ln.W2 + e0 + u * NTH] = v[u];
+    }
+    for (int e = threadIdx.x; e < 16 * ln.ldh; e += NTH) {
         const int row = e / ln.ldh, c = e - row * ln.ldh;
         float v = 0.f;
         if (NET) { if (e < H) v = P[oW3 + e]; }
@@ -503,7 +520,7 @@
     return s;
 }
 
-template <int H, int NET, int ST, bool PUB = false, bool PK = false>
+template <int H, int NET, int ST, bool PUB = false, bool PK = false, int HV = 1>
 __device__ __forceinline__ void ppo_update_net(
     float *lds, const float *__restrict__ P, const float *__restrict__ img, const Dims &d, const float *__restrict__ obs,
     const int32_t *__restrict__ act, const float *__restrict__ logp_old, const float *__restrict__ adv,
@@ -513,15 +530,25 @@
 #define NSTAMP(k) do { if (stamps && blockIdx.x == 0 && threadIdx.x == 0) stamps[16 + 24 * NET + (k)] = (long long)wall_clock64(); } while (0)
     NSTAMP(0);
     if (stamps && threadIdx.x == 0 && blockIdx.x < 256) stamps[1024 + 2 * (blockIdx.x + 256 * NET)] = (long long)wall_clock64();
-    const LayN<H> ln(d);
+    static_assert(HV == 1 || (HV == 2 && !PUB), "one tile per workgroup pass, or two side by side");
+    const int tid = HV == 2 ? (int)(threadIdx.x & (NT - 1)) : (int)threadIdx.x, half = HV == 2 ? (int)(threadIdx.x >> 8) : 0;
+    LayN<H> ln(d);
+    const PairEx<H> ex(ln, d.nJ);
+    if (HV == 2 && half) {
+        const int o = ln.total - ln.X;
+        ln.X += o; ln.H1 += o; ln.H2 += o; ln.OUT += o; ln.D3 += o; ln.D2 += o; ln.D1 += o;
+    }
     const POff<H> po(d.D, d.A);
-    const int64_t n_tiles = (M + R - 1) / R;
+    const int64_t n_tiles = (M + R - 1) / R, n_units = (n_tiles + HV - 1) / HV;
+    auto tile_of = [&](int64_t u) -> int64_t { return u * HV + half; };
+    auto ld_row0 = [&](int64_t t) -> int64_t { return HV == 2 && t >= n_tiles ? 0 : t * R; };
+    auto ld_M = [&](int64_t t) -> int64_t { return HV == 2 && t >= n_tiles ? 0 : M; };
     float xr[kXRegs];
     struct RowIn { int a_idx; float adv, logp_old, ret, v_old; } rin;
-    auto row_id = [&](int64_t row0) -> int64_t {
-        const int64_t i = row0 + (threadIdx.x >> 4);
-        const int64_t v = perm ? perm[i < M ? i : row0] : first + i;
-        return i < M ? v : -1;
+    auto row_id = [&](int64_t row0, int64_t Mv) -> int64_t {
+        const int64_t i = row0 + (tid >> 4);
+        const int64_t v = perm ? perm[i < Mv ? i : row0] : first + i;
+        return i < Mv ? v : -1;
     };
     auto prefetch_row = [&](int64_t src) {
         const int64_t s0 = src >= 0 ? src : 0;
@@ -538,57 +565,61 @@
         }
     };
     auto prefetch_packed = [&](int64_t t) {
-        const float *rec = packed + t * pack_rec_words(d.D);
+        const bool have = HV == 1 || t < n_tiles;
+        const float *rec = packed + (have ? t : 0) * pack_rec_words(d.D);
 #pragma unroll
         for (int it = 0; it < kXRegs; ++it) {
-            const int e = threadIdx.x + it * NT, r = e / d.ld1, c = e - r * d.ld1;
+            const int e = tid + it * NT, r = e / d.ld1, c = e - r * d.ld1;
             const bool ok = e < R * d.ld1 && c < d.D;
             const float v = rec[ok ? r * d.D + c : 0];
-            xr[it] = ok ? v : 0.f;
-        }
-        const float *row = rec + R * d.D + (threadIdx.x >> 4);
+            xr[it] = ok && have ? v : 0.f;
+        }
+        const float *row = rec + R * d.D + (tid >> 4);
         rin.a_idx = 0; rin.adv = 0.f; rin.logp_old = 0.f; rin.ret = 0.f; rin.v_old = 0.f;
         if (NET == 0) {
-            rin.a_idx = __float_as_int(row[0]); rin.logp_old = row[R]; rin.adv = row[2 * R];
+            const float a_ = row[0], lp_ = row[R], ad_ = row[2 * R];
+            rin.a_idx = have ? __float_as_int(a_) : 0; rin.logp_old = have ? lp_ : 0.f; rin.adv = have ? ad_ : 0.f;
         } else {
-            rin.ret = row[3 * R];
+            const float r_ = row[3 * R];
+            rin.ret = have ? r_ : 0.f;
             const float vo_ = row[4 * R];
-            rin.v_old = cfg.value_clip ? vo_ : 0.f;
+            rin.v_old = cfg.value_clip && have ? vo_ : 0.f;
         }
     };
+    const int64_t t0 = tile_of(blockIdx.x), row0_0 = ld_row0(t0), M_0 = ld_M(t0);
     if constexpr (PK) {
         static_assert(R == kPackRows, "a record is one tile");
-        prefetch_packed(blockIdx.x);
-        NetImageRegs<H> wq;
+        prefetch_packed(t0);
+        NetImageRegs<H, HV * NT> wq;
         const Lay<H> ly_img(d, true);
-        stage_net_image_load<H, NET>(wq, ly_img, d, img);
+        stage_net_image_load<H, NET, HV * NT>(wq, ly_img, d, img);
         __builtin_amdgcn_sched_barrier(0);
-        stage_net_image_store<H, NET>(lds, wq, ln, d);
-    } else if (perm && img && (int64_t)blockIdx.x < n_tiles) {
+        stage_net_image_store<H, NET, HV * NT>(lds, wq, ln, d);
+    } else if (perm && img && (int64_t)blockIdx.x < n_units) {
         int64_t xs[kXRegs], id0[kXRegs + 1];
-        prefetch_tile_ids_load<1>(id0, d, perm, first, (int64_t)blockIdx.x * R, M);
-        NetImageRegs<H> wq;
+        prefetch_tile_ids_load<1>(id0, d, perm, first, row0_0, M_0, tid);
+        NetImageRegs<H, HV * NT> wq;
         const Lay<H> ly_img(d, true);
-        stage_net_image_load<H, NET>(wq, ly_img, d, img);
+        stage_net_image_load<H, NET, HV * NT>(wq, ly_img, d, img);
         __builtin_amdgcn_sched_barrier(0);
         unsigned ok;
-        const int64_t rsrc = prefetch_tile_ids_done_nb(xs, ok, id0, d, (int64_t)blockIdx.x * R, M);
+        const int64_t rsrc = prefetch_tile_ids_done_nb(xs, ok, id0, d, row0_0, M_0, tid);
         prefetch_tile_vals_nb(xr, xs, ok, obs);
         prefetch_row(rsrc);
         __builtin_amdgcn_sched_barrier(0);
-        stage_net_image_store<H, NET>(lds, wq, ln, d);
+        stage_net_image_store<H, NET, HV * NT>(lds, wq, ln, d);
     } else {
         int64_t xs[kXRegs];
-        if ((int64_t)blockIdx.x < n_tiles) {
-            prefetch_tile_ids(xs, d, perm, first, (int64_t)blockIdx.x * R, M);
-            const int64_t rsrc = row_id((int64_t)blockIdx.x * R);
+        if ((int64_t)blockIdx.x < n_units) {
+            prefetch_tile_ids(xs, d, perm, first, row0_0, M_0, tid);
+            const int64_t rsrc = row_id(row0_0, M_0);
             prefetch_tile_vals(xr, xs, obs);
             prefetch_row(rsrc);
         }
-        if (img) { const Lay<H> ly(d, true); stage_net_image<H, NET>(lds, ln, ly, d, img); }
-        else stage_net_flat<H, NET>(lds, ln, d, P);
-    }
-    const int lane = threadIdx.x & 63, w = threadIdx.x >> 6;
+        if (img) { const Lay<H> ly(d, true); stage_net_image<H, NET, HV * NT>(lds, ln, ly, d, img); }
+        else stage_net_flat<H, NET, HV * NT>(lds, ln, d, P);
+    }
+    const int lane = tid & 63, w = tid >> 6;
     const int r16 = lane & 15, kq = lane >> 4;
     const float invM = 1.0f / (float)M;
     float a_mean = 0.f, a_std = 1.f;
@@ -615,10 +646,10 @@
                     const int row = kq * 4 + r;
                     if (row < d.A) slab_store<ST>(g_W3[r], &S[po.aW3 + row * H + 16 * w + r16]);
                 }
-                if (threadIdx.x < d.A) slab_store<ST>(g_b3, &S[po.ab3 + threadIdx.x]);
+                if (tid < d.A) slab_store<ST>(g_b3, &S[po.ab3 + tid]);
             } else {
-                if (threadIdx.x < H) slab_store<ST>(g_W3c, &S[po.cW3 + threadIdx.x]);
-                if (threadIdx.x == 0) slab_store<ST>(g_b3, &S[po.cb3]);
+                if (tid < H) slab_store<ST>(g_W3c, &S[po.cW3 + tid]);
+                if (tid == 0) slab_store<ST>(g_b3, &S[po.cb3]);
             }
         }
     };
@@ -629,7 +660,7 @@
             for (int r = 0; r < 4; ++r)
 #pragma unroll
                 for (int jb = 0; jb < 4; ++jb) slab_store<ST>(g_W2[jb][r], &S[oW2 + (16 * w + kq * 4 + r) * H + 16 * jb + r16]);
-            if (threadIdx.x < H) slab_store<ST>(g_b2, &S[(NET ? po.cb2 : po.ab2) + threadIdx.x]);
+            if (tid < H) slab_store<ST>(g_b2, &S[(NET ? po.cb2 : po.ab2) + tid]);
         }
     };
     auto store_layer1 = [&]() {
@@ -642,16 +673,56 @@
                     const int c = 16 * jb + r16;
                     if (jb < d.nJ && c < d.D) slab_store<ST>(g_W1[jb][r], &S[oW1 + (16 * w + kq * 4 + r) * d.D + c]);
                 }
-            if (threadIdx.x < H) slab_store<ST>(g_b1, &S[(NET ? po.cb1 : po.ab1) + threadIdx.x]);
-        }
+            if (tid < H) slab_store<ST>(g_b1, &S[(NET ? po.cb1 : po.ab1) + tid]);
+        }
+    };
+    auto ex_put_out = [&]() {
+        if (NET == 0) {
+            *reinterpret_cast<f4 *>(lds + ex.W3 + 4 * tid) = g_W3;
+            if (tid < 16) lds[ex.B3 + tid] = g_b3;
+        } else {
+            if (tid < H) lds[ex.W3 + tid] = g_W3c;
+            if (tid == 0) lds[ex.B3] = g_b3;
+        }
+    };
+    auto ex_add_out = [&]() {
+        if (NET == 0) {
+            g_W3 += *reinterpret_cast<const f4 *>(lds + ex.W3 + 4 * tid);
+            if (tid < 16) g_b3 += lds[ex.B3 + tid];
+        } else {
+            if (tid < H) g_W3c += lds[ex.W3 + tid];
+            if (tid == 0) g_b3 += lds[ex.B3];
+        }
+    };
+    auto ex_put_layer2 = [&]() {
+#pragma unroll
+        for (int jb = 0; jb < 4; ++jb) *reinterpret_cast<f4 *>(lds + ex.W2 + 4 * (jb * NT + tid)) = g_W2[jb];
+        if (tid < H) lds[ex.B2 + tid] = g_b2;
+    };
+    auto ex_add_layer2 = [&]() {
+#pragma unroll
+        for (int jb = 0; jb < 4; ++jb) g_W2[jb] += *reinterpret_cast<const f4 *>(lds + ex.W2 + 4 * (jb * NT + tid));
+        if (tid < H) g_b2 += lds[ex.B2 + tid];
+    };
+    auto ex_put_layer1 = [&]() {
+#pragma unroll
+        for (int jb = 0; jb < kMaxJ; ++jb)
+            if (jb < d.nJ) *reinterpret_cast<f4 *>(lds + ex.W1 + 4 * (jb * NT + tid)) = g_W1[jb];
+        if (tid < H) lds[ex.B1 + tid] = g_b1;
+    };
+    auto ex_add_layer1 = [&]() {
+#pragma unroll
+        for (int jb = 0; jb < kMaxJ; ++jb)
+            if (jb < d.nJ) g_W1[jb] += *reinterpret_cast<const f4 *>(lds + ex.W1 + 4 * (jb * NT + tid));
+        if (tid < H) g_b1 += lds[ex.B1 + tid];
     };
     bool stored = false;
     NSTAMP(1);
-    for (int64_t t = blockIdx.x; t < n_tiles; t += gridDim.x) {
-        const int64_t row0 = t * R;
-        const bool last_tile = t + gridDim.x >= n_tiles;
-        __syncthreads();
-        commit_tile_x(lds, ln.X, d, xr);
+    for (int64_t u = blockIdx.x; u < n_units; u += gridDim.x) {
+        const int64_t t = tile_of(u), row0 = t * R;
+        const bool last_tile = u + gridDim.x >= n_units;
+        __syncthreads();
+        commit_tile_x(lds, ln.X, d, xr, tid);
         const RowIn cur = rin;
         __syncthreads();
         NSTAMP(2);
@@ -691,15 +762,15 @@
 #pragma unroll
                 for (int r = 0; r < 4; ++r) lds[ln.OUT + (kq * 4 + r) * ln.ldo + r16] = acc[r] + b;
             }
-        } else if (threadIdx.x < R) {
-            const float sv = fmaf_chain_ahead<H>(lds + ln.H2 + threadIdx.x * ln.ldh, lds + ln.W3);
-            lds[ln.OUT + threadIdx.x * ln.ldo + 16] = sv + lds[ln.B3];
+        } else if (tid < R) {
+            const float sv = fmaf_chain_ahead<H>(lds + ln.H2 + tid * ln.ldh, lds + ln.W3);
+            lds[ln.OUT + tid * ln.ldo + 16] = sv + lds[ln.B3];
         }
         __syncthreads();
         NSTAMP(5);
 
         {
-            const int r = threadIdx.x >> 4, j = threadIdx.x & 15;
+            const int r = tid >> 4, j = tid & 15;
             const int64_t i = row0 + r;
             float *d3 = lds + ln.D3 + r * ln.ldo;
             float dl = 0.f, dv = 0.f;
@@ -715,7 +786,7 @@
                     const float p = ex / s;
                     const float h = row16_sum(on ? -p * l : 0.f);
                     const int a_idx = cur.a_idx;
-                    const float logp = __shfl(l, (threadIdx.x & 48) + a_idx, 64);
+                    const float logp = __shfl(l, (tid & 48) + a_idx, 64);
                     float a = cur.adv;
                     if (cfg.adv_norm) a = (a - a_mean) / (a_std + 1e-8f);
                     float ratio, obj, g_ratio;
@@ -767,11 +838,12 @@
         __syncthreads();
         NSTAMP(6);
 
-        if (t + gridDim.x < n_tiles) {
-            if constexpr (PK) prefetch_packed(t + gridDim.x);
+        if (u + gridDim.x < n_units) {
+            const int64_t tn = tile_of(u + gridDim.x);
+            if constexpr (PK) prefetch_packed(tn);
             else {
-                prefetch_tile_x(xr, d, obs, perm, first, (t + gridDim.x) * R, M);
-                prefetch_row(row_id((t + gridDim.x) * R));
+                prefetch_tile_x(xr, d, obs, perm, first, ld_row0(tn), ld_M(tn), tid);
+                prefetch_row(row_id(ld_row0(tn), ld_M(tn)));
             }
         }
         if (NET == 0) {
@@ -792,10 +864,10 @@
                 const int row = kq * 4 + r;
                 lds[ln.D2 + row * ln.ldh + col] = lds[ln.H2 + row * ln.ldh + col] > 0.f ? acc[r] : 0.f;
             }
-            if (!PUB && threadIdx.x < 16) g_b3 += column_sum(lds + ln.D3 + threadIdx.x, ln.ldo);
+            if (!PUB && tid < 16) g_b3 += column_sum(lds + ln.D3 + tid, ln.ldo);
         } else {
             static_assert(NT == 4 * H && R == 16, "one column per lane, four rows per wave");
-            const int j = threadIdx.x & (H - 1);
+            const int j = tid & (H - 1);
             float d4[4], h4[4], dv[R], hcol[R];
 #pragma unroll
             for (int k = 0; k < 4; ++k) { d4[k] = lds[ln.D3 + (4 * k + w) * ln.ldo + 16]; h4[k] = lds[ln.H2 + (4 * k + w) * ln.ldh + j]; }
@@ -812,7 +884,7 @@
 #pragma unroll
                 for (int r = 0; r < R; ++r) s = fmaf(dv[r], hcol[r], s);
                 g_W3c += s;
-                if (threadIdx.x == 0) {
+                if (tid == 0) {
                     float sb = 0.f;
 #pragma unroll
                     for (int r = 0; r < R; ++r) sb += dv[r];
@@ -820,8 +892,14 @@
                 }
             }
         }
-        if (last_tile) { store_out_layer(); stored = true; }
-        __syncthreads();
+        if (HV == 1) {
+            if (last_tile) { store_out_layer(); stored = true; }
+        } else if (last_tile && half) ex_put_out();
+        __syncthreads();
+        if (HV == 2 && last_tile) {
+            if (!half) { ex_add_out(); store_out_layer(); }
+            stored = true;
+        }
         NSTAMP(7);
         {
             const float *dA = lds + ln.D2 + kq * ln.ldh + 16 * w + r16;
@@ -832,8 +910,10 @@
 #pragma unroll
                     for (int k0 = 0; k0 < R; k0 += 4) g_W2[jb] = mfma(dA[k0 * ln.ldh], hB[k0 * ln.ldh], g_W2[jb]);
                 }
-                if (threadIdx.x < H) g_b2 += column_sum(lds + ln.D2 + threadIdx.x, ln.ldh);
-                if (last_tile) store_layer2();
+                if (tid < H) g_b2 += column_sum(lds + ln.D2 + tid, ln.ldh);
+                if (HV == 1) {
+                    if (last_tile) store_layer2();
+                } else if (last_tile && half) ex_put_layer2();
             }
             f4 acc = zero;
             const float *dR = lds + ln.D2 + r16 * ln.ldh + kq;
@@ -848,10 +928,11 @@
             }
         }
         __syncthreads();
+        if (HV == 2 && last_tile && !half) { ex_add_layer2(); store_layer2(); }
         NSTAMP(8);
         if constexpr (PUB) {
             float *pub = slabs + ((int64_t)t * 2 + NET) * pub_floats<H>(d.ld1);
-            const int pr = threadIdx.x >> 4, pc = (threadIdx.x & 15) * 4;
+            const int pr = tid >> 4, pc = (tid & 15) * 4;
             const int src[4] = {ln.H1, ln.H2, ln.D2, ln.D1};
 #pragma unroll
             for (int m = 0; m < 4; ++m) {
@@ -859,8 +940,8 @@
                 const float2 a1 = *reinterpret_cast<const float2 *>(lds + src[m] + pr * ln.ldh + pc + 2);
                 __builtin_nontemporal_store(f4{a0.x, a0.y, a1.x, a1.y}, reinterpret_cast<f4 *>(pub + m * R * H + pr * H + pc));
             }
-            for (int e = threadIdx.x; e < R * d.ld1; e += NT) __builtin_nontemporal_store(lds[ln.X + e], pub + 4 * R * H + e);
-            for (int e = threadIdx.x; e < R * ln.ldo; e += NT) __builtin_nontemporal_store(lds[ln.D3 + e], pub + 4 * R * H + R * d.ld1 + e);
+            for (int e = tid; e < R * d.ld1; e += NT) __builtin_nontemporal_store(lds[ln.X + e], pub + 4 * R * H + e);
+            for (int e = tid; e < R * ln.ldo; e += NT) __builtin_nontemporal_store(lds[ln.D3 + e], pub + 4 * R * H + R * d.ld1 + e);
         } else
         {
             const float *dA = lds + ln.D1 + kq * ln.ldh + 16 * w + r16;
@@ -872,22 +953,39 @@
                     for (int k0 = 0; k0 < R; k0 += 4) g_W1[jb] = mfma(dA[k0 * ln.ldh], xB[k0 * d.ld1], g_W1[jb]);
                 }
             }
-            if (threadIdx.x < H) g_b1 += column_sum(lds + ln.D1 + threadIdx.x, ln.ldh);
+            if (tid < H) g_b1 += column_sum(lds + ln.D1 + tid, ln.ldh);
         }
     }
 
     NSTAMP(9);
-    if (!stored) { store_out_layer(); store_layer2(); }
-    store_layer1();
+    if (HV == 1) {
+        if (!stored) { store_out_layer(); store_layer2(); }
+        store_layer1();
+    } else {
+        if (half) {
+            if (!stored) { ex_put_out(); ex_put_layer2(); }
+            ex_put_layer1();
+        }
+        __syncthreads();
+        if (!half) {
+            if (!stored) { ex_add_out(); store_out_layer(); ex_add_layer2(); store_layer2(); }
+            ex_add_layer1();
+            store_layer1();
+        }
+    }
     NSTAMP(10);
     {
-        __shared__ double s_red[2][NT / 64];
+        __shared__ double s_red[2][HV * NT / 64];
         const double a = wave_sum(s_a), b = wave_sum(s_b);
-        if (lane == 0) { s_red[0][w] = a; s_red[1][w] = b; }
-        __syncthreads();
-        if (threadIdx.x == 0) {
-            const double ta = s_red[0][0] + s_red[0][1] + s_red[0][2] + s_red[0][3];
-            const double tb = s_red[1][0] + s_red[1][1] + s_red[1][2] + s_red[1][3];
+        if (lane == 0) { s_red[0][4 * half + w] = a; s_red[1][4 * half + w] = b; }
+        __syncthreads();
+        if (tid == 0 && !half) {
+            double ta = s_red[0][0] + s_red[0][1] + s_red[0][2] + s_red[0][3];
+            double tb = s_red[1][0] + s_red[1][1] + s_red[1][2] + s_red[1][3];
+            if (HV == 2) {
+                ta += s_red[0][4] + s_red[0][5] + s_red[0][6] + s_red[0][7];
+                tb += s_red[1][4] + s_red[1][5] + s_red[1][6] + s_red[1][7];
+            }
             if (NET == 0) {
                 loss_partial[4 * blockIdx.x + 0] = ta;
                 loss_partial[4 * blockIdx.x + 2] = tb;
@@ -919,6 +1017,32 @@
     else
         ppo_update_net<H, 1, ST, PUB, PK>(lds, P, img, d, obs, act, logp_old, adv, returns, v_s_old, perm, first, M, adv_stats, cfg,
                                           slabs, loss_partial, stamps, packed);
+}
+
+template <int H, int DS, bool PK>
+__global__ __launch_bounds__(2 * NT) void ppo_update_pair_kernel(
+    const float *__restrict__ P, const float *__restrict__ img, Dims d_arg, const float *__restrict__ obs,
+    const int32_t *__restrict__ act, const float *__restrict__ logp_old, const float *__restrict__ adv,
+    const float *__restrict__ returns, const float *__restrict__ v_s_old, const int64_t *__restrict__ perm, int64_t first,
+    int64_t M, const float *__restrict__ adv_stats, LossCfg cfg, float *__restrict__ slabs,
+    double *__restrict__ loss_partial, int64_t *__restrict__ opt_step_dev, long long *stamps, const float *__restrict__ packed) {
+    extern __shared__ float lds[];
+    const Dims d = DS ? dims_const(DS, 5) : d_arg;
+    if (opt_step_dev && blockIdx.x == 0 && blockIdx.y == 0 && threadIdx.x == 0) *opt_step_dev += 1;
+    if (blockIdx.y == 0)
+        ppo_update_net<H, 0, 0, false, PK, 2>(lds, P, img, d, obs, act, logp_old, adv, returns, v_s_old, perm, first, M, adv_stats, cfg,
+                                              slabs, loss_partial, stamps, packed);
+    else
+        ppo_update_net<H, 1, 0, false, PK, 2>(lds, P, img, d, obs, act, logp_old, adv, returns, v_s_old, perm, first, M, adv_stats, cfg,
+                                              slabs, loss_partial, stamps, packed);
+}
+
+__global__ __launch_bounds__(256) void pair_fold_kernel(const float *__restrict__ a, const float *__restrict__ b, float *__restrict__ out,
+                                                        int64_t n, const double *__restrict__ pa, const double *__restrict__ pb,
+                                                        double *__restrict__ pout, int64_t np) {
+    const int64_t i = (int64_t)blockIdx.x * 256 + threadIdx.x;
+    if (i < n) out[i] = a[i] + b[i];
+    if (i < np) pout[i] = pa[i] + pb[i];
 }
 
 __global__ __launch_bounds__(256) void update_finalize_kernel(const double *__restrict__ partial, int n_blocks,
@@ -1055,11 +1179,19 @@
 extern "C" int tsm_debug_update_variant_get(void) { return g_update_variant; }
 extern "C" int tsm_debug_slab_store_get(void) { return g_slab_store; }
 
+constexpr int kPairMaxGrid = 128;
+static bool update_pair_form(int64_t M, int32_t n_blocks) {
+    const int64_t n_tiles = ceil_div(M, R);
+    return n_tiles >= 2 && n_blocks <= (n_tiles + 1) / 2 && n_blocks <= kPairMaxGrid;
+}
+
 TSM_EXPORT int tsm_ppo_update_grid(int64_t M, int32_t max_blocks) {
     const int64_t n_tiles = ceil_div(M > 0 ? M : 1, R);
     int64_t g;
-    if (n_tiles <= 256) g = n_tiles;
-    else if (n_tiles < 1024) g = (n_tiles + 1) / 2 < 256 ? (n_tiles + 1) / 2 : 256;
+    if (n_tiles <= 128) g = n_tiles;
+    else if (n_tiles <= 256) g = (n_tiles + 1) / 2;
+    else if (n_tiles <= 512) g = (n_tiles + 3) / 4;
+    else if (n_tiles < 1024) g = 256;
     else g = 384;
     if (max_blocks > 0 && g > max_blocks) g = max_blocks;
     return (int)g;
@@ -1098,6 +1230,12 @@
     static bool attr_set = false;
     if (!attr_set) {
         TSM_HIP(tsm_allow_max_lds(reinterpret_cast<const void *>(ppo_update_kernel<64>)));
+        TSM_HIP(tsm_allow_max_lds(reinterpret_cast<const void *>(ppo_update_pair_kernel<64, 18, true>)));
+        TSM_HIP(tsm_allow_max_lds(reinterpret_cast<const void *>(ppo_update_pair_kernel<64, 18, false>)));
+        TSM_HIP(tsm_allow_max_lds(reinterpret_cast<const void *>(ppo_update_pair_kernel<64, 16, true>)));
+        TSM_HIP(tsm_allow_max_lds(reinterpret_cast<const void *>(ppo_update_pair_kernel<64, 16, false>)));
+        TSM_HIP(tsm_allow_max_lds(reinterpret_cast<const void *>(ppo_update_pair_kernel<64, 0, true>)));
+        TSM_HIP(tsm_allow_max_lds(reinterpret_cast<const void *>(ppo_update_pair_kernel<64, 0, false>)));
         attr_set = true;
     }
     hipStream_t st = tsm_stream(stream);
@@ -1109,10 +1247,19 @@
                            (size_t)ln.total * sizeof(float), st, params, param_image, d, obs, act, logp_old, adv, returns,
                            v_s_old, perm, first_row, M, adv_stats, cfg, grad_slabs_out, loss_partial_out, opt_step_dev, g_tsm_stamps,
                            (const float *)nullptr);
-    } else if (g_update_variant == 0) {
+    } else if (g_update_variant == 0 || g_update_variant == 3) {
         const LayN<64> ln(d);
         const bool spec = d.A == 5 && !tsm_opt(TSM_OPT_GENERIC);
         const bool pk = packed && param_image && g_slab_store == 0;
+        if (g_slab_store == 0 && g_update_variant == 0 && update_pair_form(M, n_blocks)) {
+            const size_t bytes = (size_t)PairEx<64>(ln, d.nJ).total * sizeof(float);
+            auto pair = (spec && d.D == 18) ? (pk ? ppo_update_pair_kernel<64, 18, true> : ppo_update_pair_kernel<64, 18, false>)
+                        : (spec && d.D == 16) ? (pk ? ppo_update_pair_kernel<64, 16, true> : ppo_update_pair_kernel<64, 16, false>)
+                        : pk ? ppo_update_pair_kernel<64, 0, true> : ppo_update_pair_kernel<64, 0, false>;
+            hipLaunchKernelGGL(pair, dim3((unsigned)n_blocks, 2), dim3(2 * NT), bytes, st, params, param_image, d, obs, act,
+                               logp_old, adv, returns, v_s_old, perm, first_row, M, adv_stats, cfg, grad_slabs_out,
+                               loss_partial_out, opt_step_dev, g_tsm_stamps, pk ? packed : nullptr);
+        } else {
         auto kern = g_slab_store == 1 ? ppo_update_split_kernel<64, 1, 0>
                     : g_slab_store == 2 ? ppo_update_split_kernel<64, 2, 0>
                     : (spec && d.D == 18) ? (pk ? ppo_update_split_kernel<64, 0, 18, false, true>
@@ -1124,11 +1271,33 @@
                            (size_t)ln.total * sizeof(float), st, params, param_image, d, obs, act, logp_old, adv, returns,
                            v_s_old, perm, first_row, M, adv_stats, cfg, grad_slabs_out, loss_partial_out, opt_step_dev, g_tsm_stamps,
                            pk ? packed : nullptr);
+        }
+    } else if (update_pair_form(M, n_blocks)) {
+        static float *tmp = nullptr;
+        static size_t tmp_bytes = 0;
+        const int64_t n = (int64_t)n_blocks * POff<64>(d.D, d.A).total, np = (int64_t)n_blocks * 4;
+        const size_t need = (size_t)(2 * n) * sizeof(float) + (size_t)(2 * np) * sizeof(double);
+        if (need > tmp_bytes) {
+            if (tmp) TSM_HIP(hipFree(tmp));
+            tmp = nullptr; tmp_bytes = 0;
+            TSM_HIP(hipMalloc(reinterpret_cast<void **>(&tmp), need));
+            tmp_bytes = need;
+        }
+        double *ptmp = reinterpret_cast<double *>(tmp);
+        float *stmp = tmp + 4 * np;
+        for (int par = 0; par < 2; ++par) {
+            hipLaunchKernelGGL((ppo_update_kernel<64>), dim3((unsigned)n_blocks), dim3(NT), shmem, st, params, param_image, d,
+                               obs, act, logp_old, adv, returns, v_s_old, perm, first_row, M, adv_stats, cfg, stmp + par * n,
+                               ptmp + par * np, par ? nullptr : opt_step_dev, g_tsm_stamps, 2, par);
+            TSM_LAUNCH_CHECK();
+        }
+        hipLaunchKernelGGL(pair_fold_kernel, dim3((unsigned)ceil_div(n, 256)), dim3(256), 0, st, stmp, stmp + n, grad_slabs_out, n,
+                           ptmp, ptmp + np, loss_partial_out, np);
     } else {
         hipLaunchKernelGGL((ppo_update_kernel<64>), dim3((unsigned)n_blocks), dim3(NT), shmem, st, params, param_image, d,
                            obs, act,
                            logp_old, adv, returns, v_s_old, perm, first_row, M, adv_stats, cfg, grad_slabs_out,
-                           loss_partial_out, opt_step_dev, g_tsm_stamps);
+                           loss_partial_out, opt_step_dev, g_tsm_stamps, 1, 0);
     }
     TSM_LAUNCH_CHECK();
     if (scalars_out) {
diff --git a/tianshou_marl_amd/csrc/mlp_tile.h b/tianshou_marl_amd/csrc/mlp_tile.h
--- a/tianshou_marl_amd/csrc/mlp_tile.h
+++ b/tianshou_marl_amd/csrc/mlp_tile.h
@@ -278,41 +278,41 @@
 
 template <int HAS_PERM = -1>
 __device__ __forceinline__ void prefetch_tile_ids_load(int64_t (&id)[kXRegs + 1], const Dims &d, const int64_t *__restrict__ perm,
-                                                       int64_t first, int64_t row0, int64_t M) {
-    const int64_t ir = row0 + (threadIdx.x >> 4);
+                                                       int64_t first, int64_t row0, int64_t M, int tid = threadIdx.x) {
+    const int64_t ir = row0 + (tid >> 4);
     if (HAS_PERM == 1 || (HAS_PERM == -1 && perm)) {
 #pragma unroll
         for (int it = 0; it < kXRegs; ++it) {
-            const int e = threadIdx.x + it * NT, r = e / d.ld1;
+            const int e = tid + it * NT, r = e / d.ld1;
             const int64_t i = row0 + r;
             id[it] = perm[(e < R * d.ld1 && i < M) ? i : row0];
         }
         id[kXRegs] = perm[ir < M ? ir : row0];
     } else {
 #pragma unroll
-        for (int it = 0; it < kXRegs; ++it) id[it] = first + row0 + (threadIdx.x + it * NT) / d.ld1;
+        for (int it = 0; it < kXRegs; ++it) id[it] = first + row0 + (tid + it * NT) / d.ld1;
         id[kXRegs] = first + ir;
     }
 }
 __device__ __forceinline__ int64_t prefetch_tile_ids_done(int64_t (&xs)[kXRegs], const int64_t (&id)[kXRegs + 1], const Dims &d,
-                                                          int64_t row0, int64_t M) {
-#pragma unroll
-    for (int it = 0; it < kXRegs; ++it) {
-        const int e = threadIdx.x + it * NT, r = e / d.ld1, c = e - r * d.ld1;
+                                                          int64_t row0, int64_t M, int tid = threadIdx.x) {
+#pragma unroll
+    for (int it = 0; it < kXRegs; ++it) {
+        const int e = tid + it * NT, r = e / d.ld1, c = e - r * d.ld1;
         xs[it] = (e < R * d.ld1 && c < d.D && row0 + r < M) ? id[it] * d.D + c : -1;
     }
-    return row0 + (threadIdx.x >> 4) < M ? id[kXRegs] : -1;
+    return row0 + (tid >> 4) < M ? id[kXRegs] : -1;
 }
 __device__ __forceinline__ int64_t prefetch_tile_ids_done_nb(int64_t (&xs)[kXRegs], unsigned &ok, const int64_t (&id)[kXRegs + 1],
-                                                             const Dims &d, int64_t row0, int64_t M) {
+                                                             const Dims &d, int64_t row0, int64_t M, int tid = threadIdx.x) {
     ok = 0;
 #pragma unroll
     for (int it = 0; it < kXRegs; ++it) {
-        const int e = threadIdx.x + it * NT, r = e / d.ld1, c = e - r * d.ld1;
+        const int e = tid + it * NT, r = e / d.ld1, c = e - r * d.ld1;
         xs[it] = id[it] * d.D + (c < d.D ? c : 0);
         ok |= (unsigned)(e < R * d.ld1 && c < d.D && row0 + r < M) << it;
     }
-    return row0 + (threadIdx.x >> 4) < M ? id[kXRegs] : -1;
+    return row0 + (tid >> 4) < M ? id[kXRegs] : -1;
 }
 __device__ __forceinline__ void prefetch_tile_vals_nb(float (&xr)[kXRegs], const int64_t (&xs)[kXRegs], unsigned ok,
                                                       const float *__restrict__ obs) {
@@ -324,10 +324,10 @@
 }
 __device__ __forceinline__ void prefetch_tile_ids(int64_t (&xs)[kXRegs], const Dims &d,
                                                   const int64_t *__restrict__ perm, int64_t first, int64_t row0,
-                                                  int64_t M) {
+                                                  int64_t M, int tid = threadIdx.x) {
     int64_t id[kXRegs + 1];
-    prefetch_tile_ids_load(id, d, perm, first, row0, M);
-    (void)prefetch_tile_ids_done(xs, id, d, row0, M);
+    prefetch_tile_ids_load(id, d, perm, first, row0, M, tid);
+    (void)prefetch_tile_ids_done(xs, id, d, row0, M, tid);
 }
 
 __device__ __forceinline__ void prefetch_tile_vals(float (&xr)[kXRegs], const int64_t (&xs)[kXRegs],
@@ -341,16 +341,16 @@
 
 __device__ __forceinline__ void prefetch_tile_x(float (&xr)[kXRegs], const Dims &d, const float *__restrict__ obs,
                                                 const int64_t *__restrict__ perm, int64_t first, int64_t row0,
-                                                int64_t M) {
+                                                int64_t M, int tid = threadIdx.x) {
     int64_t xs[kXRegs];
-    prefetch_tile_ids(xs, d, perm, first, row0, M);
+    prefetch_tile_ids(xs, d, perm, first, row0, M, tid);
     prefetch_tile_vals(xr, xs, obs);
 }
 
-__device__ __forceinline__ void commit_tile_x(float *lds, int X, const Dims &d, const float (&xr)[kXRegs]) {
-#pragma unroll
-    for (int it = 0; it < kXRegs; ++it) {
-        const int e = threadIdx.x + it * NT;
+__device__ __forceinline__ void commit_tile_x(float *lds, int X, const Dims &d, const float (&xr)[kXRegs], int tid = threadIdx.x) {
+#pragma unroll
+    for (int it = 0; it < kXRegs; ++it) {
+        const int e = tid + it * NT;
         if (e < R * d.ld1) lds[X + e] = xr[it];
     }
 }
```

Result: slower. 160.8 million env-steps/s (-3.4%).
